# xiaojino/RUArt

Hardware: AMD Instinct MI355X
Metric: VQA samples/sec fwd+bwd (B=64, q=30, ocr=100) (higher is better)
Workload: dtype f16 MFMA + block-scaled fp8 (e4m3) MFMA correction, f32 accumulate / residual stream; 1 GPU; RUArt training step, synthetic ST-VQA-shaped batch: B=64/GPU, q=30 words, 100 OCR items, 36 objects, bert-base 12x768 frozen, SDNet trunk fwd+bwd, Adamax; global_batch=64, real_wordpieces_per_batch=42738, parallelism=dp1, mode=train

## Files before the change

### include/ruart_hip.h

```cpp
#ifndef RUART_HIP_H
#define RUART_HIP_H
#include <stddef.h>
#include <stdint.h>

#ifdef __cplusplus
extern "C" {
#endif

#define RUART_DT_F32 0
#define RUART_DT_BF16 1
#define RUART_DT_F16 2
#define RUART_ACT_NONE 0
#define RUART_ACT_GELU 1
#define RUART_ACT_RELU 2

const char* ruart_version(void);

int ruart_gemm_16_nt(const void* A, int lda, const void* W, int ldw, const float* bias, const void* residual, int ldr,
                     int residual_dtype, void* C, int ldc, int out_dtype, int M, int N, int K, int act, int in_dtype,
                     void* stream);
size_t ruart_gemm_16_tail_ws_bytes(int M, int N, int K, int cus);
int ruart_gemm_16_nt_ws(const void* A, int lda, const void* W, int ldw, const float* bias, const void* residual, int ldr, int residual_dtype,
                        void* C, int ldc, int out_dtype, int M, int N, int K, int act, int in_dtype, void* tail_ws, size_t tail_ws_bytes, int cus,
                        void* stream);
int ruart_gemm_16c_nt(const void* A16, const void* A8, int lda, const void* W16, const void* W8, int ldw, const float* bias,
                      const float* residual, int ldr, void* C, int ldc, void* C8, int M, int N, int K, int act, void* stream);
int ruart_f16c_shifts(int* out4);
int ruart_gemm_16c_set_dual(int on);
int ruart_gemm_16c_nt_sel(const void* A16, const void* A8, int lda, const void* W16, const void* W8, int ldw, const float* bias,
                          const float* residual, int ldr, void* C, int ldc, void* C8, int M, int N, int K, int act, int corr, void* stream);
size_t ruart_gemm_16c_tail_ws_bytes(int M, int N, int K, int cus);
int ruart_gemm_16c_nt_ws(const void* A16, const void* A8, int lda, const void* W16, const void* W8, int ldw, const float* bias,
                         const float* residual, int ldr, void* C, int ldc, void* C8, int M, int N, int K, int act, int corr, void* tail_ws,
                         size_t tail_ws_bytes, int cus, void* stream);
int ruart_gemm_16_nt_gelu2(const void* A, int lda, const void* W, int ldw, const float* bias, void* H16, void* G16, int ldc, int M, int N, int K,
                           int in_dtype, void* stream);
size_t ruart_gemm_16_nt_gelu_bwd_ws_floats(int M, int N);
int ruart_gemm_16_nt_gelu_bwd(const void* dY_bf16, int lda, const void* Wt_bf16, int ldw, const void* H16, int ldh, void* dH_bf16, void* G_bf16,
                              int ldc, float* colpart, int M, int N, int K, void* stream);
int ruart_gemm_16_nt_splitk(const void* A, int lda, const void* W, int ldw, float* part, int ldc, int M, int N, int K, int kchunk,
                            int in_dtype, void* stream);
int ruart_gemm_16_tn_splitk(const void* P, int ldp, const void* Q, int ldq, float* part, int ldc, int M, int N, int T, int tchunk,
                            int in_dtype, void* stream);
int ruart_gemm_set_tile_order(int group_m);
int ruart_gemm_set_variant(int v);
int ruart_gemm_f32_nt(const float* A, int lda, const float* W, int ldw, const float* bias, const float* residual, int ldr,
                      float* C, int ldc, int M, int N, int K, int act, void* stream);

int ruart_prof_enable(int on);
int ruart_prof_read(double* total_ms, long long* launches, double* flops);
int ruart_prof_mark(int tag, void* stream);
int ruart_prof_timeline(float* begin_ms, float* end_ms, double* flops, int max_records, int* n_records);

int ruart_bert_embed_ln(const int* ids, const int* pos_ids, const float* word_emb, const float* pos_emb, const float* type_emb,
                        const float* gamma, const float* beta, float eps, void* out, int ldo, int out_dtype, int rows, int H,
                        void* stream);
int ruart_rows_layernorm(const float* x, int ldx, const float* gamma, const float* beta, float eps, void* out, int ldo,
                         int out_dtype, int rows, int H, void* stream);
int ruart_rows_layernorm_split(const float* x, int ldx, const float* gamma, const float* beta, float eps, float* out32, void* out16,
                               void* out8, int ldo, int rows, int H, void* stream);
int ruart_bert_embed_ln_split(const int* ids, const int* pos_ids, const float* word_emb, const float* pos_emb, const float* type_emb,
                              const float* gamma, const float* beta, float eps, float* out32, void* out16, void* out8, int ldo, int rows,
                              int H, void* stream);
int ruart_bert_attention(const void* qkv, int ld, void* ctx, int ldc, int dtype, int H, int n_heads, int n_blocks,
                         const int* blk_q0, const int* blk_q1, const int* blk_k0, const int* blk_k1, const int* tok_lo,
                         const int* tok_hi, const float* key_bias, int n_long_blocks, const int* lblk_q0, const int* lblk_q1,
                         const int* lblk_k0, const int* lblk_k1, void* stream);
int ruart_bert_attention_split(const float* qkv, int ld, void* ctx16, void* ctx8, int ldc, int H, int n_heads, int n_blocks,
                               const int* blk_q0, const int* blk_q1, const int* blk_k0, const int* blk_k1, const int* tok_lo,
                               const int* tok_hi, const float* key_bias, void* stream);
int ruart_bert_attention_split_set_heads(int heads_per_workgroup);
int ruart_bert_pool_set_variant(int cols);
int ruart_bert_pool_mix(const void* layers, long long layer_stride, int ldl, int dtype, int n_layers, const int* span_start,
                        const int* span_start_last, const int* span_len, const int* dst_row, const float* layer_w, float* out, int ldo,
                        int n_words, int H, void* stream);
int ruart_bert_pool_mix_bwd(const void* layers, long long layer_stride, int ldl, int dtype, int n_layers, const int* span_start,
                            const int* span_start_last, const int* span_len, const int* dst_row, const float* grad_out, int ldg,
                            float* partial_ws, float* grad_layer_w, int n_words, int H, void* stream);
int ruart_rows_gather(const int* rows, int n, const void* src0, long long sp0, void* dst0, long long dp0, int bytes0, const void* src1,
                      long long sp1, void* dst1, long long dp1, int bytes1, const void* src2, long long sp2, void* dst2, long long dp2,
                      int bytes2, void* stream);
int ruart_cast_f32_to_16(const float* in, void* out, int out_dtype, long long n, float scale, void* stream);

int ruart_ln_train_fwd(const float* x, int ldx, const void* res16, int ldr, const float* gamma, const float* beta, float eps, float p,
                       unsigned seed, int post, void* y16, void* pre16, float* stats, int ld16, int rows, int H, void* stream);
size_t ruart_ln_train_bwd_ws_floats(int H);
int ruart_ln_train_bwd(const float* dy, int ldy, const float* add, const float* add_scale, const void* pre16, int ld16, const float* stats,
                       const float* gamma, float p, unsigned seed, int post, float* d_res, int ldd, void* d_gemm_bf16, int ldg,
                       float* d_gamma, float* d_beta, float* d_bias, int accumulate, float* ws, int rows, int H, void* stream);
typedef struct {
  const float* w;
  void* out16;
  void* outT_bf16;
  int ldw, ld16, ldT, rows, cols;
  float scale;
} ruart_wprep_item;
int ruart_weight_prep_batch(const ruart_wprep_item* items, int n, void* stream);
int ruart_weight_prep(const float* w, int ldw, float scale, void* out16, int ld16, void* outT_bf16, int ldT, int rows, int cols, void* stream);
size_t ruart_colsum_f32_ws_floats(int rows, int cols);
int ruart_colsum_f32(const float* x, int ld, int rows, int cols, float* out, int accumulate, float* ws, void* stream);
int ruart_colsum_f32_rows(const float* part, int rows, int ld, int cols, float* out, int accumulate, void* stream);
int ruart_gelu_bwd_rows(void* d_bf16, const void* h16, int ld, void* g_bf16, float* colpart, int M, int N, void* stream);
int ruart_f16_to_bf16(const void* in16, void* out_bf16, long long n, void* stream);
int ruart_colsum_bf16(const void* x_bf16, int ld, int rows, int cols, float* out, int accumulate, float* ws, void* stream);
int ruart_transpose16(const void* in, int ldi, void* out, int ldo, int rows, int cols, int f16_to_bf16, void* stream);
int ruart_splitk_reduce(const float* part, long long slab_floats, int nz, float* C, long long n, float scale, int accumulate, void* stream);
int ruart_mix_rows(const void* layers16, long long layer_stride, int ld, int n_layers, const float* w, float* out, int ldo, int rows, int H,
                   void* stream);
int ruart_mix_rows_bwd(const void* layers16, long long layer_stride, int ld, int n_layers, const float* g, int ldg, float* d_w, float* ws,
                       int rows, int H, void* stream);
int ruart_rows_ln_to_16(const float* y, long long layer_stride, int ldy, const float* ln_stats, long long stats_stride, const float* ln_gamma,
                        const float* ln_beta, void* out16, long long out_stride, int ldo, int n_layers, int n_tokens, int rows, int H,
                        void* stream);
int ruart_attn_train_fwd(const void* qkv16, int ld, void* ctx16, int ldc, int H, int n_heads, int n_blocks, const int* blk_q0,
                         const int* blk_q1, const int* tok_lo, float p_drop, unsigned seed, void* stream);
int ruart_attn_train_bwd(const void* qkv16, int ld, const void* dctx_bf16, int ldc, void* dqkv_bf16, int ldd, int H, int n_heads, int n_blocks,
                         const int* blk_q0, const int* blk_q1, const int* tok_lo, float p_drop, unsigned seed, float* bias_part, void* stream);
int ruart_attn_train_fwd_long(const void* qkv16, int ld, void* ctx16, int ldc, int H, int n_heads, int n_chunks, const int* chunk_q0,
                              const int* chunk_q1, const int* chunk_k0, const int* chunk_k1, float p_drop, unsigned seed, float* lse2,
                              void* stream);
int ruart_attn_train_bwd_long(const void* qkv16, int ld, const void* dctx_bf16, int ldc, void* dqkv_bf16, int ldd, int H, int n_heads,
                              int n_chunks, const int* chunk_q0, const int* chunk_q1, const int* chunk_k0, const int* chunk_k1, const int* chunk_first, float p_drop, unsigned seed, const float* lse2, float* delta_ws,
                              float* scale_ws, float* bias_part, void* stream);

typedef struct {
  int hidden, n_heads, n_layers, intermediate, dtype;
  float ln_eps;
  const float *word_emb, *pos_emb, *type_emb, *emb_ln_g, *emb_ln_b;
  const void* const* w_qkv;
  const float* const* b_qkv;
  const void* const* w_ao;    const float* const* b_ao;
  const float* const* ln1_g;  const float* const* ln1_b;
  const void* const* w_ff1;   const float* const* b_ff1;
  const void* const* w_ff2;   const float* const* b_ff2;
  const float* const* ln2_g;  const float* const* ln2_b;
  int f32_gemm;
  int corr8;
  const void* const* w8_qkv;
  const void* const* w8_ao;
  const void* const* w8_ff1;
  const void* const* w8_ff2;
  int tail_cus;
  int ln_fold;
  const float* const* fold_c_qkv;
  const float* const* fold_c_ff1;
  const float* fold_s_qkv;
  const float* fold_s_ff1;
} ruart_bert_model;

typedef struct {
  int n_tokens;
  int n_rows;
  const int* ids;
  const int* pos_ids;
  int n_blocks;
  const int *blk_q0, *blk_q1, *blk_k0, *blk_k1, *tok_lo, *tok_hi;
  const float* key_bias;
  int n_long_blocks;
  const int *lblk_q0, *lblk_q1, *lblk_k0, *lblk_k1;
  int n_last_rows;
  const int* last_rows;
} ruart_bert_batch;

size_t ruart_bert_workspace_bytes(const ruart_bert_model* m, int n_rows);
int ruart_bert_set_correction(int qkv, int ao, int ff1, int ff2, unsigned long long layer_mask);
int ruart_bert_forward(const ruart_bert_model* m, const ruart_bert_batch* b, void* layers_out, void* workspace,
                       size_t workspace_bytes, void* stream);

size_t ruart_bert_workspace_bytes_folded(const ruart_bert_model* m, int n_rows);
int ruart_bert_forward_folded(const ruart_bert_model* m, const ruart_bert_batch* b, void* layers_pre, float* ln_stats, void* workspace,
                              size_t workspace_bytes, void* stream);
int ruart_gemm_16c_nt_fold(const void* A16, const void* A8, int lda, const void* W16, const void* W8, int ldw, const float* bias, int kind,
                           const float* in_part, int in_np, const float* colc, float wscale, const float* residual, int ldr,
                           const float* res_part, int res_np, const float* res_gamma, const float* res_beta, void* C, int ldc, void* C16,
                           void* C8, float* out_part, int M, int N, int K, int stat_len, float eps, void* stream);
int ruart_gemm_16_nt_fold(const void* A, int lda, const void* W, int ldw, const float* bias, int kind, const float* in_part, int in_np,
                          const float* colc, float wscale, const void* residual, int ldr, const float* res_part, int res_np,
                          const float* res_gamma, const float* res_beta, void* C, int ldc, float* out_part, int M, int N, int K, int stat_len,
                          float eps, int dtype, void* stream);
int ruart_rows_stats_finish(const float* part, int np, int rows, float inv_h, float eps, float* stats, void* stream);
int ruart_bert_pool_mix_ln(const float* layers_pre, long long layer_stride, int ldl, int n_layers, const float* ln_stats,
                           long long stats_stride, const float* ln_gamma, const float* ln_beta, const int* span_start,
                           const int* span_start_last, const int* span_len, const int* dst_row, const float* layer_w, float* out, int ldo,
                           int n_words, int H, void* stream);
int ruart_bert_pool_ln_set_variant(int reg_tables);
int ruart_bert_pool_mix_ln_bwd(const float* layers_pre, long long layer_stride, int ldl, int n_layers, const float* ln_stats,
                               long long stats_stride, const float* ln_gamma, const float* ln_beta, const int* span_start,
                               const int* span_start_last, const int* span_len, const int* dst_row, const float* grad_out, int ldg,
                               float* partial_ws, float* grad_layer_w, int n_words, int H, void* stream);

int ruart_attn_fwd(const float* pa, const float* pk, const float* v, const unsigned char* mask, const float* diag, int diag_len,
                   int relu, float* out, float* probs, int B, int L1, int L2, int h, int D3, void* stream);
int ruart_attn_bwd(const float* pa, const float* pk, const float* v, const float* probs, const float* grad_out, const float* diag,
                   int diag_len, int relu, float* grad_pa, float* grad_pk, float* grad_v, float* grad_diag_partial,
                   float* ds_ws , int B, int L1, int L2, int h, int D3, void* stream);
int ruart_attn_set_prefetch(int on);
int ruart_attn_fwd_pscale(const float* pa, const float* pk, const float* v, const unsigned char* mask, const float* diag, int diag_len,
                          int relu, const float* prob_scale, float* out, float* probs, int B, int L1, int L2, int h, int D3,
                          void* stream);
int ruart_attn_bwd_pscale(const float* pa, const float* pk, const float* v, const float* probs, const float* grad_out, const float* diag,
                          int diag_len, int relu, const float* prob_scale, float* grad_pa, float* grad_pk, float* grad_v,
                          float* grad_diag_partial, float* ds_ws, int B, int L1, int L2, int h, int D3, void* stream);

int ruart_whole_ln_fwd(const float* x, float* y, float* stats, float* ws, long long n, float eps, void* stream);
int ruart_whole_ln_bwd(const float* y, const float* grad_y, const float* stats, float* grad_x, float* ws, long long n,
                       void* stream);

int ruart_whole_ln_blocks(void);
int ruart_whole_ln_partials(const float* x, const float* x2, float* part, long long n, void* stream);
int ruart_whole_ln_var_global(const float* x, long long n, const float* part_all, int world, long long n_total, float* part2,
                              void* stream);
int ruart_whole_ln_apply_global(const float* x, float* y, long long n, float eps, const float* part_all, const float* part2_all,
                                int world, long long n_total, float* stats, void* stream);
int ruart_whole_ln_bwd_global(const float* y, const float* grad_y, const float* stats, float* grad_x, long long n,
                              const float* part_all, int world, long long n_total, void* stream);

int ruart_scorer_fwd(const float* x, const float* u1, const float* u2, const float* uh, const float* w, const float* bna,
                     const unsigned char* mask, float* probs, float* a_out, int B, int L, int D, int ES, int mask_flag, void* stream);
int ruart_scorer_bwd(const float* x, const float* u1, const float* u2, const float* uh, const float* w, const float* probs,
                     const float* a_in, const float* gprobs, float* gx, float* gu1, float* gu2, float* guh, float* gw_part,
                     float* gb_part, int B, int L, int D, int ES, void* stream);

int ruart_scorer_heads_fwd(const float* x, const float* u1, const float* u2, const float* uh, const float* w, const float* bh,
                           const unsigned char* mask, float* probs, float* a_out, int B, int L, int D, int ES, int H, int n_front,
                           int mask_flag, void* stream);
int ruart_scorer_heads_bwd(const float* x, const float* u1, const float* u2, const float* uh, const float* w, const float* probs,
                           const float* a_in, const float* gprobs, float* gx, float* gu1, float* gu2, float* guh, float* gw_part,
                           float* gb_part, int B, int L, int D, int ES, int H, int n_front, void* stream);

int ruart_lstm_set_variant(int variant);
int ruart_lstm_ws_bytes(int h, int ndir, size_t* bytes);
int ruart_lstm_fwd(const float* xproj, const float* w_hh, float* y, float* gates, float* cells, float* hprev, int B, int T, int h,
                   int ndir, void* ws, size_t ws_bytes, void* stream);
int ruart_lstm_bwd(const float* grad_y, const float* w_hh, const float* gates, const float* cells, float* grad_xproj, int B,
                   int T, int h, int ndir, void* ws, size_t ws_bytes, void* stream);

int ruart_lstm_pack_params(const float* w_ih, const float* w_ih_r, const float* b_ih, const float* b_hh, const float* b_ih_r,
                           const float* b_hh_r, const float* w_hh, const float* w_hh_r, float* w, float* b, float* whh, int G, int K, int h,
                           void* stream);

int ruart_rows_scale(const float* x, int ldx, const float* mask, int ldm, const long long* row_of, float* out, int ldo, int rows, int D,
                     void* stream);
int ruart_lstm_cell_fwd(const float* pre, const float* h_prev, const float* c_prev, float* h_out, float* c_out, float* acts,
                        int n_active, int n_rows, int h, void* stream);
int ruart_lstm_cell_bwd(const float* grad_h, const float* grad_c, const float* acts, const float* c_prev, const float* c_out,
                        float* grad_pre, float* grad_h_prev, float* grad_c_prev, int n_active, int n_rows, int h, void* stream);

int ruart_embedding_bwd_sorted(const float* grad_out, const int* order, const int* seg_start, const int* seg_row, int n_seg, int D,
                               float* grad_weight, void* stream);
int ruart_embedding_bwd_split(const float* grad_out, const int* order, const int* sub_start, int n_sub, const int* row_first, const int* row_id,
                              int n_rows, int D, float* ws, float* grad_weight, void* stream);

int ruart_phoc_table(const unsigned char* chars, const int* offsets, int n_words, float* out, int ldo, int* status, void* stream);

#define RUART_EDIT_MAX_LEN 128
int ruart_edit_distance_pairs(const int32_t* chars, int n_chars, const int32_t* str_off, int n_str, const int32_t* pair_a,
                              const int32_t* pair_b, int n_pairs, int32_t* dist, int32_t* equal, void* stream);

int ruart_grad_norm_clip(const float* const* grads, const int* c_tensor, const int* c_start, const int* c_count, int n_chunks,
                         float max_norm, float* partial, float* norm_coef, const float* extra_sq, void* stream);
int ruart_adamax_step(float* const* params, const float* const* grads, float* const* exp_avg, float* const* exp_inf, const int* c_tensor,
                      const int* c_start, const int* c_count, int n_chunks, const float* norm_coef, const float* clr, float beta1,
                      float beta2, float eps, void* stream);
int ruart_adam_step(float* const* params, const float* const* grads, float* const* exp_avg, float* const* exp_avg_sq, const int* c_tensor,
                    const int* c_start, const int* c_count, int n_chunks, const float* norm_coef, const float* tab, float beta1,
                    float beta2, float eps, void* stream);

int ruart_set_nan_flag(int* flag);

int ruart_gemm_x3_plan(int M, int N, int K, int a_k_contiguous , int b_k_contiguous , int* splitk,
                       size_t* ws_bytes);
int ruart_gemm_x3(const float* A, long long sam, long long sak, const float* B, long long sbk, long long sbn, const float* bias,
                  const float* residual, int ldr, int act, float* C, int ldc, int M, int N, int K, float* ws, size_t ws_bytes,
                  const unsigned char* a_keep, const unsigned char* b_keep, float keep_scale, const float* c_scale, int rows_per_scale_row,
                  void* stream);
typedef struct {
  const float* A;
  const float* B;
  float* C;
  int lda, ldb, ldc, M, N, K, accumulate;
} ruart_x3_tn_problem;
size_t ruart_gemm_x3_tn_grouped_ws(const ruart_x3_tn_problem* probs, int n);
int ruart_gemm_x3_tn_grouped(const ruart_x3_tn_problem* probs, int n, float* ws, size_t ws_bytes, void* stream);
int ruart_gemm_x1(const float* A, long long sam, long long sak, const float* B, long long sbk, long long sbn, const float* bias,
                  const float* residual, int ldr, int act, float* C, int ldc, int M, int N, int K, float* ws, size_t ws_bytes,
                  const unsigned char* a_keep, const unsigned char* b_keep, float keep_scale, const float* c_scale, int rows_per_scale_row,
                  void* stream);

int ruart_gemm_bf16_tn(const float* A, long long sak_rows, const float* B, long long sbk_rows, float* C, int ldc, int M, int N, int K,
                       float* ws, size_t ws_bytes, void* stream);

int ruart_stream_create_cu_masked(int n_cus, void** stream_out);
int ruart_stream_create_priority(int priority, void** stream_out);
int ruart_stream_destroy(void* stream);

#ifdef __cplusplus
}
#endif
#endif
```

### ruart_amd/csrc/sdnet_attention.hip

```cpp
#include <cstdlib>
#include "common.h"
#include "ruart_hip.h"

#define CH 64
#define LDA_ 66
#define LDB_ 80
#define NTW 6
#define ATTN_MAX_L2 384

int* ruart_nan_flag_ptr = nullptr;

__device__ __forceinline__ f32x4_t mma16(const float* As, int lda, const float* Bs, int sbk, int sbj, int Kc, f32x4_t acc) {
  const int lane = threadIdx.x & 63, r = lane & 15, q = lane >> 4;
  for (int kk = 0; kk < Kc; kk += 4) acc = __builtin_amdgcn_mfma_f32_16x16x4f32(As[r * lda + kk + q], Bs[(kk + q) * sbk + r * sbj], acc, 0, 0, 0);
  return acc;
}

struct Act {
  int relu;
  const float* diag;
  int diag_len;
  __device__ __forceinline__ float operator()(float v, int col) const {
    if (relu) v = fmaxf(v, 0.f);
    if (diag_len == 1) v *= diag[0];
    else if (diag_len > 1) v *= diag[col];
    return v;
  }
};
__device__ __forceinline__ Act no_act() { return Act{0, nullptr, 0}; }

template <int U>
__device__ __forceinline__ void stage_u(float* dst, int ldd, int nr_pad, const float* src, int ld, int r0, int rows, int c0, int cols, Act act) {
  const int total = nr_pad * CH;
  for (int e0 = threadIdx.x; e0 < total; e0 += U * blockDim.x) {
    float v[U], dv[U];
    unsigned ok = 0;
#pragma unroll
    for (int u = 0; u < U; ++u) {
      const int e = e0 + u * blockDim.x;
      const int r = e / CH, c = e % CH;
      const int gr = r0 + r, gc = c0 + c;
      if (e < total && gr < rows && gc < cols) ok |= 1u << u;
      v[u] = src[(size_t)min(gr, rows - 1) * ld + min(gc, cols - 1)];
    }
    if (act.diag_len > 1) {
#pragma unroll
      for (int u = 0; u < U; ++u) dv[u] = act.diag[min(c0 + (e0 + u * (int)blockDim.x) % CH, cols - 1)];
    } else {
      const float d1 = act.diag_len == 1 ? act.diag[0] : 1.f;
#pragma unroll
      for (int u = 0; u < U; ++u) dv[u] = d1;
    }
#pragma unroll
    for (int u = 0; u < U; ++u) {
      const int e = e0 + u * blockDim.x;
      float x = v[u];
      if (act.relu) x = fmaxf(x, 0.f);
      x *= dv[u];
      if (e < total) dst[(e / CH) * ldd + (e % CH)] = ((ok >> u) & 1u) ? x : 0.f;
    }
  }
}
__device__ __forceinline__ void stage(float* dst, int ldd, int nr_pad, const float* src, int ld, int r0, int rows, int c0, int cols,
                                      Act act = Act{0, nullptr, 0}) {
  if (nr_pad <= 16) stage_u<4>(dst, ldd, nr_pad, src, ld, r0, rows, c0, cols, act);
  else if (nr_pad <= 32) stage_u<8>(dst, ldd, nr_pad, src, ld, r0, rows, c0, cols, act);
  else stage_u<16>(dst, ldd, nr_pad, src, ld, r0, rows, c0, cols, act);
}
__device__ __forceinline__ void stage_t16(float* dst, int ldd, const float* src, int ld, int r0, int rows, int c0, int cols,
                                          const float* mul = nullptr) {
  float v[4], m[4];
  unsigned ok = 0;
#pragma unroll
  for (int u = 0; u < 4; ++u) {
    const int e = threadIdx.x + u * 256;
    const int c = e & 15, r = e >> 4;
    const int gr = r0 + r, gc = c0 + c;
    if (gr < rows && gc < cols) ok |= 1u << u;
    const size_t at = (size_t)min(gr, rows - 1) * ld + min(gc, cols - 1);
    v[u] = src[at];
    m[u] = mul ? mul[at] : 1.f;
  }
#pragma unroll
  for (int u = 0; u < 4; ++u) {
    const int e = threadIdx.x + u * 256;
    dst[(e & 15) * ldd + (e >> 4)] = ((ok >> u) & 1u) ? v[u] * m[u] : 0.f;
  }
}

__device__ __forceinline__ int lds_probs_stride(int L2p) { return ((L2p + 31) / 32) * 32 + 2; }

extern __shared__ __attribute__((aligned(16))) float dsm[];

__global__ __launch_bounds__(256) void attn_fwd_kernel(const float* __restrict__ a, const float* __restrict__ k,
                                                       const float* __restrict__ v, const unsigned char* __restrict__ mask,
                                                       float* __restrict__ out, float* __restrict__ probs, int L1, int L2, int h,
                                                       int D3, int* __restrict__ nan_flag, int relu, const float* __restrict__ diag,
                                                       int diag_len, const float* __restrict__ pscale) {
  const int b = blockIdx.y, i0 = blockIdx.x * 16;
  const int lane = threadIdx.x & 63, wave = threadIdx.x >> 6;
  const int L2p = (L2 + 15) & ~15, ldS = lds_probs_stride(L2p);
  float* a_s = dsm;
  float* S_s = a_s + 16 * LDA_;
  float* kv_s = S_s + 16 * ldS;
  const float* ab = a + (size_t)b * L1 * h;
  const float* kb = k + (size_t)b * L2 * h;
  const float* vb = v + (size_t)b * L2 * D3;
  const int ntile = L2p / 16;

  f32x4_t acc[NTW];
#pragma unroll
  for (int t = 0; t < NTW; ++t) acc[t] = (f32x4_t){0.f, 0.f, 0.f, 0.f};
  for (int c0 = 0; c0 < h; c0 += CH) {
    __syncthreads();
    stage(a_s, LDA_, 16, ab, h, i0, L1, c0, h, Act{relu, diag, diag_len});
    stage(kv_s, LDA_, L2p, kb, h, 0, L2, c0, h, Act{relu, nullptr, 0});
    __syncthreads();
    const int kc = min(CH, (h - c0 + 3) & ~3);
#pragma unroll
    for (int t = 0; t < NTW; ++t) {
      const int jt = wave + 4 * t;
      if (jt < ntile) acc[t] = mma16(a_s, LDA_, kv_s + jt * 16 * LDA_, 1, LDA_, kc, acc[t]);
    }
  }
#pragma unroll
  for (int t = 0; t < NTW; ++t) {
    const int jt = wave + 4 * t;
    if (jt < ntile) {
#pragma unroll
      for (int r = 0; r < 4; ++r) S_s[((lane >> 4) * 4 + r) * ldS + jt * 16 + (lane & 15)] = acc[t][r];
    }
  }
  __syncthreads();
  {
    const int row = threadIdx.x >> 4, c = threadIdx.x & 15;
    const unsigned char* mb = mask + (size_t)b * L2;
    float* Sr = S_s + row * ldS;
    float mx = -INFINITY;
    for (int j = c; j < L2; j += 16) {
      const float s = mb[j] ? Sr[j] : -INFINITY;
      Sr[j] = s;
      mx = fmaxf(mx, s);
    }
#pragma unroll
    for (int o = 8; o > 0; o >>= 1) mx = fmaxf(mx, __shfl_xor(mx, o, 64));
    float sum = 0.f;
    for (int j = c; j < L2; j += 16) {
      const float e = expf(Sr[j] - mx);
      Sr[j] = e;
      sum += e;
    }
#pragma unroll
    for (int o = 8; o > 0; o >>= 1) sum += __shfl_xor(sum, o, 64);
    const float inv = 1.0f / sum;
    const bool live = (i0 + row) < L1;
    bool bad = false;
    for (int j = c; j < L2p; j += 16) {
      const float p = (j < L2) ? Sr[j] * inv : 0.f;
      const float ps = (pscale && live && j < L2) ? pscale[((size_t)b * L1 + i0 + row) * L2 + j] : 1.f;
      Sr[j] = live ? p * ps : 0.f;
      bad |= live && !(p == p);
      if (probs && live && j < L2) probs[((size_t)b * L1 + i0 + row) * L2 + j] = p;
    }
    if (bad && nan_flag) atomicOr(nan_flag, 1);
  }
  for (int d0 = 0; d0 < D3; d0 += CH) {
    __syncthreads();
    stage(kv_s, LDB_, L2p, vb, D3, 0, L2, d0, D3);
    __syncthreads();
    f32x4_t o = {0.f, 0.f, 0.f, 0.f};
    o = mma16(S_s, ldS, kv_s + wave * 16, LDB_, 1, L2p, o);
    const int d = d0 + wave * 16 + (lane & 15);
#pragma unroll
    for (int r = 0; r < 4; ++r) {
      const int i = i0 + (lane >> 4) * 4 + r;
      if (i < L1 && d < D3) out[((size_t)b * L1 + i) * D3 + d] = o[r];
    }
  }
}

__global__ __launch_bounds__(256) void attn_bwd_q_kernel(const float* __restrict__ k, const float* __restrict__ v,
                                                         const float* __restrict__ probs, const float* __restrict__ gout,
                                                         float* __restrict__ grad_a, float* __restrict__ dS, int L1, int L2, int h,
                                                         int D3, const float* __restrict__ pa, int relu,
                                                         const float* __restrict__ diag, int diag_len,
                                                         float* __restrict__ grad_diag, const float* __restrict__ pscale) {
  const int b = blockIdx.y, i0 = blockIdx.x * 16;
  const int lane = threadIdx.x & 63, wave = threadIdx.x >> 6;
  const int L2p = (L2 + 15) & ~15, ldS = lds_probs_stride(L2p);
  float* g_s = dsm;
  float* S_s = g_s + 16 * LDA_;
  float* kv_s = S_s + 16 * ldS;
  const float* kb = k + (size_t)b * L2 * h;
  const float* vb = v + (size_t)b * L2 * D3;
  const float* gb = gout + (size_t)b * L1 * D3;
  const int ntile = L2p / 16;

  f32x4_t acc[NTW];
#pragma unroll
  for (int t = 0; t < NTW; ++t) acc[t] = (f32x4_t){0.f, 0.f, 0.f, 0.f};
  for (int c0 = 0; c0 < D3; c0 += CH) {
    __syncthreads();
    stage(g_s, LDA_, 16, gb, D3, i0, L1, c0, D3);
    stage(kv_s, LDA_, L2p, vb, D3, 0, L2, c0, D3);
    __syncthreads();
    const int kc = min(CH, (D3 - c0 + 3) & ~3);
#pragma unroll
    for (int t = 0; t < NTW; ++t) {
      const int jt = wave + 4 * t;
      if (jt < ntile) acc[t] = mma16(g_s, LDA_, kv_s + jt * 16 * LDA_, 1, LDA_, kc, acc[t]);
    }
  }
#pragma unroll
  for (int t = 0; t < NTW; ++t) {
    const int jt = wave + 4 * t;
    if (jt < ntile) {
#pragma unroll
      for (int r = 0; r < 4; ++r) S_s[((lane >> 4) * 4 + r) * ldS + jt * 16 + (lane & 15)] = acc[t][r];
    }
  }
  __syncthreads();
  {
    const int row = threadIdx.x >> 4, c = threadIdx.x & 15;
    const bool live = (i0 + row) < L1;
    const float* Pr = probs + ((size_t)b * L1 + (live ? i0 + row : 0)) * L2;
    float* Sr = S_s + row * ldS;
    float dot = 0.f;
    if (pscale && live) {
      const float* Mr = pscale + ((size_t)b * L1 + i0 + row) * L2;
      for (int j = c; j < L2; j += 16) Sr[j] *= Mr[j];
    }
    for (int j = c; j < L2; j += 16) dot += Sr[j] * Pr[j];
#pragma unroll
    for (int o = 8; o > 0; o >>= 1) dot += __shfl_xor(dot, o, 64);
    for (int j = c; j < L2p; j += 16) {
      float d = 0.f;
      if (live && j < L2) {
        const float p = Pr[j];
        d = p * (Sr[j] - dot);
        dS[((size_t)b * L1 + i0 + row) * L2 + j] = d;
      }
      Sr[j] = d;
    }
  }
  for (int d0 = 0; d0 < h; d0 += CH) {
    __syncthreads();
    stage(kv_s, LDB_, L2p, kb, h, 0, L2, d0, h, Act{relu, nullptr, 0});
    __syncthreads();
    f32x4_t o = {0.f, 0.f, 0.f, 0.f};
    o = mma16(S_s, ldS, kv_s + wave * 16, LDB_, 1, L2p, o);
    const int d = d0 + wave * 16 + (lane & 15);
    float gd = 0.f;
    const float dsc = (d < h) ? (diag_len == 1 ? diag[0] : (diag_len > 1 ? diag[d] : 1.f)) : 0.f;
#pragma unroll
    for (int r = 0; r < 4; ++r) {
      const int i = i0 + (lane >> 4) * 4 + r;
      if (i < L1 && d < h) {
        const size_t at = ((size_t)b * L1 + i) * h + d;
        float g = o[r];
        if (pa) {
          const float pv = pa[at];
          gd += g * (relu ? fmaxf(pv, 0.f) : pv);
          g = (relu && pv <= 0.f) ? 0.f : g * dsc;
        }
        grad_a[at] = g;
      }
    }
    if (grad_diag) {
      gd += __shfl_xor(gd, 16, 64);
      gd += __shfl_xor(gd, 32, 64);
      if ((lane >> 4) == 0 && d < h) grad_diag[((size_t)b * gridDim.x + blockIdx.x) * h + d] = gd;
    }
  }
}

__device__ __forceinline__ void tn_product(const float* X, int L1, int L2, int j0, const float* Y, int N, float* C, float* xt_s,
                                           float* y_s, Act yact, const float* out_gate, const float* xmul = nullptr) {
  const int lane = threadIdx.x & 63, wave = threadIdx.x >> 6;
  for (int n0 = 0; n0 < N; n0 += CH) {
    f32x4_t o = {0.f, 0.f, 0.f, 0.f};
    for (int r0 = 0; r0 < L1; r0 += CH) {
      __syncthreads();
      stage_t16(xt_s, LDA_, X, L2, r0, L1, j0, L2, xmul);
      stage(y_s, LDB_, CH, Y, N, r0, L1, n0, N, yact);
      __syncthreads();
      const int kc = min(CH, (L1 - r0 + 3) & ~3);
      o = mma16(xt_s, LDA_, y_s + wave * 16, LDB_, 1, kc, o);
    }
    const int n = n0 + wave * 16 + (lane & 15);
#pragma unroll
    for (int r = 0; r < 4; ++r) {
      const int j = j0 + (lane >> 4) * 4 + r;
      if (j < L2 && n < N) {
        const size_t at = (size_t)j * N + n;
        C[at] = (out_gate && out_gate[at] <= 0.f) ? 0.f : o[r];
      }
    }
  }
}

__global__ __launch_bounds__(256) void attn_bwd_kv_kernel(const float* __restrict__ a, const float* __restrict__ probs,
                                                          const float* __restrict__ dS, const float* __restrict__ gout,
                                                          float* __restrict__ grad_k, float* __restrict__ grad_v, int L1, int L2, int h,
                                                          int D3, const float* __restrict__ pk, int relu,
                                                          const float* __restrict__ diag, int diag_len,
                                                          const float* __restrict__ pscale) {
  const int b = blockIdx.y, j0 = blockIdx.x * 16;
  float* xt_s = dsm;
  float* y_s = xt_s + 16 * LDA_;
  const size_t pb = (size_t)b * L1 * L2;
  tn_product(dS + pb, L1, L2, j0, a + (size_t)b * L1 * h, h, grad_k + (size_t)b * L2 * h, xt_s, y_s, Act{relu, diag, diag_len},
             (relu && pk) ? pk + (size_t)b * L2 * h : nullptr);
  tn_product(probs + pb, L1, L2, j0, gout + (size_t)b * L1 * D3, D3, grad_v + (size_t)b * L2 * D3, xt_s, y_s, no_act(), nullptr,
             pscale ? pscale + pb : nullptr);
}

template <int U, bool DIAG = false>
struct Panel {
  float v[U];
  float dv[DIAG ? U : 1];
  unsigned ok;
  __device__ __forceinline__ void load(const float* __restrict__ src, int ld, int nr_pad, int r0, int rows, int c0, int cols,
                                       const float* __restrict__ diag = nullptr, int diag_len = 0) {
    ok = 0;
    const int total = nr_pad * CH;
#pragma unroll
    for (int u = 0; u < U; ++u) {
      const int e = (int)threadIdx.x + u * 256;
      const int r = e / CH, c = e % CH;
      const int gr = r0 + r, gc = c0 + c;
      if (e < total && gr < rows && gc < cols) ok |= 1u << u;
      v[u] = src[(size_t)min(gr, rows - 1) * ld + min(gc, cols - 1)];
      if (DIAG) dv[u] = diag_len > 1 ? diag[min(gc, cols - 1)] : (diag_len == 1 ? diag[0] : 1.f);
    }
  }
  __device__ __forceinline__ void store(float* dst, int ldd, int nr_pad, int relu) const {
    const int total = nr_pad * CH;
#pragma unroll
    for (int u = 0; u < U; ++u) {
      const int e = (int)threadIdx.x + u * 256;
      float x = v[u];
      if (relu) x = fmaxf(x, 0.f);
      x *= DIAG ? dv[u] : 1.f;
      if (e < total) dst[(e / CH) * ldd + (e % CH)] = ((ok >> u) & 1u) ? x : 0.f;
    }
  }
};

template <int UK>
__global__ __launch_bounds__(256) void attn_fwd_pf_kernel(const float* __restrict__ a, const float* __restrict__ k,
                                                          const float* __restrict__ v, const unsigned char* __restrict__ mask,
                                                          float* __restrict__ out, float* __restrict__ probs, int L1, int L2, int h,
                                                          int D3, int* __restrict__ nan_flag, int relu, const float* __restrict__ diag,
                                                          int diag_len, const float* __restrict__ pscale) {
  const int b = blockIdx.y, i0 = blockIdx.x * 16;
  const int lane = threadIdx.x & 63, wave = threadIdx.x >> 6;
  const int L2p = (L2 + 15) & ~15, ldS = lds_probs_stride(L2p);
  float* a_s = dsm;
  float* S_s = a_s + 16 * LDA_;
  float* kv_s = S_s + 16 * ldS;
  const float* ab = a + (size_t)b * L1 * h;
  const float* kb = k + (size_t)b * L2 * h;
  const float* vb = v + (size_t)b * L2 * D3;
  const int ntile = L2p / 16;

  Panel<4, true> pa;
  Panel<UK> pk;
  pa.load(ab, h, 16, i0, L1, 0, h, diag, diag_len);
  pk.load(kb, h, L2p, 0, L2, 0, h);
  f32x4_t acc[NTW];
#pragma unroll
  for (int t = 0; t < NTW; ++t) acc[t] = (f32x4_t){0.f, 0.f, 0.f, 0.f};
  for (int c0 = 0; c0 < h; c0 += CH) {
    __syncthreads();
    pa.store(a_s, LDA_, 16, relu);
    pk.store(kv_s, LDA_, L2p, relu);
    {
      const bool more = c0 + CH < h;
      pa.load(ab, h, 16, i0, L1, more ? c0 + CH : 0, h, diag, diag_len);
      pk.load(more ? kb : vb, more ? h : D3, L2p, 0, L2, more ? c0 + CH : 0, more ? h : D3);
    }
    __syncthreads();
    const int kc = min(CH, (h - c0 + 3) & ~3);
#pragma unroll
    for (int t = 0; t < NTW; ++t) {
      const int jt = wave + 4 * t;
      if (jt < ntile) acc[t] = mma16(a_s, LDA_, kv_s + jt * 16 * LDA_, 1, LDA_, kc, acc[t]);
    }
  }
#pragma unroll
  for (int t = 0; t < NTW; ++t) {
    const int jt = wave + 4 * t;
    if (jt < ntile) {
#pragma unroll
      for (int r = 0; r < 4; ++r) S_s[((lane >> 4) * 4 + r) * ldS + jt * 16 + (lane & 15)] = acc[t][r];
    }
  }
  __syncthreads();
  {
    const int row = threadIdx.x >> 4, c = threadIdx.x & 15;
    const unsigned char* mb = mask + (size_t)b * L2;
    float* Sr = S_s + row * ldS;
    float mx = -INFINITY;
    for (int j = c; j < L2; j += 16) {
      const float s = mb[j] ? Sr[j] : -INFINITY;
      Sr[j] = s;
      mx = fmaxf(mx, s);
    }
#pragma unroll
    for (int o = 8; o > 0; o >>= 1) mx = fmaxf(mx, __shfl_xor(mx, o, 64));
    float sum = 0.f;
    for (int j = c; j < L2; j += 16) {
      const float e = expf(Sr[j] - mx);
      Sr[j] = e;
      sum += e;
    }
#pragma unroll
    for (int o = 8; o > 0; o >>= 1) sum += __shfl_xor(sum, o, 64);
    const float inv = 1.0f / sum;
    const bool live = (i0 + row) < L1;
    bool bad = false;
    for (int j = c; j < L2p; j += 16) {
      const float p = (j < L2) ? Sr[j] * inv : 0.f;
      const float ps = (pscale && live && j < L2) ? pscale[((size_t)b * L1 + i0 + row) * L2 + j] : 1.f;
      Sr[j] = live ? p * ps : 0.f;
      bad |= live && !(p == p);
      if (probs && live && j < L2) probs[((size_t)b * L1 + i0 + row) * L2 + j] = p;
    }
    if (bad && nan_flag) atomicOr(nan_flag, 1);
  }
  for (int d0 = 0; d0 < D3; d0 += CH) {
    __syncthreads();
    pk.store(kv_s, LDB_, L2p, 0);
    pk.load(vb, D3, L2p, 0, L2, d0 + CH < D3 ? d0 + CH : 0, D3);
    __syncthreads();
    f32x4_t o = {0.f, 0.f, 0.f, 0.f};
    o = mma16(S_s, ldS, kv_s + wave * 16, LDB_, 1, L2p, o);
    const int d = d0 + wave * 16 + (lane & 15);
#pragma unroll
    for (int r = 0; r < 4; ++r) {
      const int i = i0 + (lane >> 4) * 4 + r;
      if (i < L1 && d < D3) out[((size_t)b * L1 + i) * D3 + d] = o[r];
    }
  }
}

template <int UK>
__global__ __launch_bounds__(256) void attn_bwd_q_pf_kernel(const float* __restrict__ k, const float* __restrict__ v,
                                                            const float* __restrict__ probs, const float* __restrict__ gout,
                                                            float* __restrict__ grad_a, float* __restrict__ dS, int L1, int L2, int h,
                                                            int D3, const float* __restrict__ pa_, int relu,
                                                            const float* __restrict__ diag, int diag_len,
                                                            float* __restrict__ grad_diag, const float* __restrict__ pscale) {
  const int b = blockIdx.y, i0 = blockIdx.x * 16;
  const int lane = threadIdx.x & 63, wave = threadIdx.x >> 6;
  const int L2p = (L2 + 15) & ~15, ldS = lds_probs_stride(L2p);
  float* g_s = dsm;
  float* S_s = g_s + 16 * LDA_;
  float* kv_s = S_s + 16 * ldS;
  const float* kb = k + (size_t)b * L2 * h;
  const float* vb = v + (size_t)b * L2 * D3;
  const float* gb = gout + (size_t)b * L1 * D3;
  const int ntile = L2p / 16;

  Panel<4> pg;
  Panel<UK> pk;
  pg.load(gb, D3, 16, i0, L1, 0, D3);
  pk.load(vb, D3, L2p, 0, L2, 0, D3);
  f32x4_t acc[NTW];
#pragma unroll
  for (int t = 0; t < NTW; ++t) acc[t] = (f32x4_t){0.f, 0.f, 0.f, 0.f};
  for (int c0 = 0; c0 < D3; c0 += CH) {
    __syncthreads();
    pg.store(g_s, LDA_, 16, 0);
    pk.store(kv_s, LDA_, L2p, 0);
    {
      const bool more = c0 + CH < D3;
      pg.load(gb, D3, 16, i0, L1, more ? c0 + CH : 0, D3);
      pk.load(more ? vb : kb, more ? D3 : h, L2p, 0, L2, more ? c0 + CH : 0, more ? D3 : h);
    }
    __syncthreads();
    const int kc = min(CH, (D3 - c0 + 3) & ~3);
#pragma unroll
    for (int t = 0; t < NTW; ++t) {
      const int jt = wave + 4 * t;
      if (jt < ntile) acc[t] = mma16(g_s, LDA_, kv_s + jt * 16 * LDA_, 1, LDA_, kc, acc[t]);
    }
  }
#pragma unroll
  for (int t = 0; t < NTW; ++t) {
    const int jt = wave + 4 * t;
    if (jt < ntile) {
#pragma unroll
      for (int r = 0; r < 4; ++r) S_s[((lane >> 4) * 4 + r) * ldS + jt * 16 + (lane & 15)] = acc[t][r];
    }
  }
  __syncthreads();
  {
    const int row = threadIdx.x >> 4, c = threadIdx.x & 15;
    const bool live = (i0 + row) < L1;
    const float* Pr = probs + ((size_t)b * L1 + (live ? i0 + row : 0)) * L2;
    float* Sr = S_s + row * ldS;
    float dot = 0.f;
    if (pscale && live) {
      const float* Mr = pscale + ((size_t)b * L1 + i0 + row) * L2;
      for (int j = c; j < L2; j += 16) Sr[j] *= Mr[j];
    }
    for (int j = c; j < L2; j += 16) dot += Sr[j] * Pr[j];
#pragma unroll
    for (int o = 8; o > 0; o >>= 1) dot += __shfl_xor(dot, o, 64);
    for (int j = c; j < L2p; j += 16) {
      float d = 0.f;
      if (live && j < L2) {
        const float p = Pr[j];
        d = p * (Sr[j] - dot);
        dS[((size_t)b * L1 + i0 + row) * L2 + j] = d;
      }
      Sr[j] = d;
    }
  }
  for (int d0 = 0; d0 < h; d0 += CH) {
    __syncthreads();
    pk.store(kv_s, LDB_, L2p, relu);
    pk.load(kb, h, L2p, 0, L2, d0 + CH < h ? d0 + CH : 0, h);
    __syncthreads();
    f32x4_t o = {0.f, 0.f, 0.f, 0.f};
    o = mma16(S_s, ldS, kv_s + wave * 16, LDB_, 1, L2p, o);
    const int d = d0 + wave * 16 + (lane & 15);
    float gd = 0.f;
    const float dsc = (d < h) ? (diag_len == 1 ? diag[0] : (diag_len > 1 ? diag[d] : 1.f)) : 0.f;
#pragma unroll
    for (int r = 0; r < 4; ++r) {
      const int i = i0 + (lane >> 4) * 4 + r;
      if (i < L1 && d < h) {
        const size_t at = ((size_t)b * L1 + i) * h + d;
        float g = o[r];
        if (pa_) {
          const float pv = pa_[at];
          gd += g * (relu ? fmaxf(pv, 0.f) : pv);
          g = (relu && pv <= 0.f) ? 0.f : g * dsc;
        }
        grad_a[at] = g;
      }
    }
    if (grad_diag) {
      gd += __shfl_xor(gd, 16, 64);
      gd += __shfl_xor(gd, 32, 64);
      if ((lane >> 4) == 0 && d < h) grad_diag[((size_t)b * gridDim.x + blockIdx.x) * h + d] = gd;
    }
  }
}

struct PanelT16 {
  float v[4], m[4];
  unsigned ok;
  __device__ __forceinline__ void load(const float* __restrict__ src, int ld, int r0, int rows, int c0, int cols, const float* __restrict__ mul) {
    ok = 0;
#pragma unroll
    for (int u = 0; u < 4; ++u) {
      const int e = (int)threadIdx.x + u * 256;
      const int c = e & 15, r = e >> 4;
      const int gr = r0 + r, gc = c0 + c;
      if (gr < rows && gc < cols) ok |= 1u << u;
      const size_t at = (size_t)min(gr, rows - 1) * ld + min(gc, cols - 1);
      v[u] = src[at];
      m[u] = mul ? mul[at] : 1.f;
    }
  }
  __device__ __forceinline__ void store(float* dst, int ldd) const {
#pragma unroll
    for (int u = 0; u < 4; ++u) {
      const int e = (int)threadIdx.x + u * 256;
      dst[(e & 15) * ldd + (e >> 4)] = ((ok >> u) & 1u) ? v[u] * m[u] : 0.f;
    }
  }
};

__device__ __forceinline__ void tn_product_pf(const float* X, int L1, int L2, int j0, const float* Y, int N, float* C, float* xt_s,
                                              float* y_s, Act yact, const float* out_gate, const float* xmul) {
  const int lane = threadIdx.x & 63, wave = threadIdx.x >> 6;
  const int nr = (L1 + CH - 1) / CH, nn = (N + CH - 1) / CH, steps = nr * nn;
  PanelT16 px;
  Panel<16, true> py;
  px.load(X, L2, 0, L1, j0, L2, xmul);
  py.load(Y, N, CH, 0, L1, 0, N, yact.diag, yact.diag_len);
  f32x4_t o = {0.f, 0.f, 0.f, 0.f};
  int ri = 0, ni = 0;
  for (int s = 0; s < steps; ++s) {
    const int r0 = ri * CH, n0 = ni * CH;
    __syncthreads();
    px.store(xt_s, LDA_);
    py.store(y_s, LDB_, CH, yact.relu);
    int rn = ri + 1, nx = ni;
    if (rn == nr) { rn = 0; nx = ni + 1; }
    if (nx == nn) { rn = 0; nx = 0; }
    px.load(X, L2, rn * CH, L1, j0, L2, xmul);
    py.load(Y, N, CH, rn * CH, L1, nx * CH, N, yact.diag, yact.diag_len);
    __syncthreads();
    const int kc = min(CH, (L1 - r0 + 3) & ~3);
    o = mma16(xt_s, LDA_, y_s + wave * 16, LDB_, 1, kc, o);
    if (ri == nr - 1) {
      const int n = n0 + wave * 16 + (lane & 15);
#pragma unroll
      for (int r = 0; r < 4; ++r) {
        const int j = j0 + (lane >> 4) * 4 + r;
        if (j < L2 && n < N) {
          const size_t at = (size_t)j * N + n;
          C[at] = (out_gate && out_gate[at] <= 0.f) ? 0.f : o[r];
        }
      }
      o = (f32x4_t){0.f, 0.f, 0.f, 0.f};
    }
    ri = rn;
    ni = nx;
  }
}

__global__ __launch_bounds__(256) void attn_bwd_kv_pf_kernel(const float* __restrict__ a, const float* __restrict__ probs,
                                                             const float* __restrict__ dS, const float* __restrict__ gout,
                                                             float* __restrict__ grad_k, float* __restrict__ grad_v, int L1, int L2, int h,
                                                             int D3, const float* __restrict__ pk, int relu,
                                                             const float* __restrict__ diag, int diag_len,
                                                             const float* __restrict__ pscale) {
  const int b = blockIdx.y, j0 = blockIdx.x * 16;
  float* xt_s = dsm;
  float* y_s = xt_s + 16 * LDA_;
  const size_t pb = (size_t)b * L1 * L2;
  tn_product_pf(dS + pb, L1, L2, j0, a + (size_t)b * L1 * h, h, grad_k + (size_t)b * L2 * h, xt_s, y_s, Act{relu, diag, diag_len},
                (relu && pk) ? pk + (size_t)b * L2 * h : nullptr, nullptr);
  tn_product_pf(probs + pb, L1, L2, j0, gout + (size_t)b * L1 * D3, D3, grad_v + (size_t)b * L2 * D3, xt_s, y_s, no_act(), nullptr,
                pscale ? pscale + pb : nullptr);
}

#define WLN_BLOCKS 256
__device__ __forceinline__ float grid_partial_total(const float* part, float* red) {
  float s = (threadIdx.x < WLN_BLOCKS) ? part[threadIdx.x] : 0.f;
  return block_sum<4>(s, red);
}

#define WLN_FOR4(n4, ...)                                                                          \
  for (long long i_ = blockIdx.x * 256LL + threadIdx.x; i_ < (n4); i_ += 4LL * 256 * WLN_BLOCKS) { \
    long long ix_[4];                                                                              \
    bool ok_[4];                                                                                   \
    _Pragma("unroll") for (int u_ = 0; u_ < 4; ++u_) {                                             \
      const long long j_ = i_ + (long long)u_ * 256 * WLN_BLOCKS;                                  \
      ok_[u_] = j_ < (n4);                                                                         \
      ix_[u_] = ok_[u_] ? j_ : (n4) - 1;                                                           \
    }                                                                                              \
    __VA_ARGS__                                                                                    \
  }
__device__ __forceinline__ bool wln_vec_ok(const void* a, const void* b, const void* c, long long n) {
  return ((n & 3) == 0) && (((reinterpret_cast<uintptr_t>(a) | reinterpret_cast<uintptr_t>(b) | reinterpret_cast<uintptr_t>(c)) & 15) == 0) && n >= 4;
}

__global__ __launch_bounds__(256) void wln_sum_kernel(const float* __restrict__ x, const float* __restrict__ x2, long long n,
                                                      float* __restrict__ part) {
  __shared__ float red[4];
  float s = 0.f, t = 0.f;
  if (wln_vec_ok(x, x2, nullptr, n)) {
    const f32x4_t* x4 = reinterpret_cast<const f32x4_t*>(x);
    const f32x4_t* y4 = reinterpret_cast<const f32x4_t*>(x2);
    const long long n4 = n >> 2;
    if (x2) {
      WLN_FOR4(n4, f32x4_t a[4], b[4];
               _Pragma("unroll") for (int u = 0; u < 4; ++u) { a[u] = x4[ix_[u]]; b[u] = y4[ix_[u]]; }
               _Pragma("unroll") for (int u = 0; u < 4; ++u) if (ok_[u]) {
                 s += (a[u][0] + a[u][1]) + (a[u][2] + a[u][3]);
                 t += (a[u][0] * b[u][0] + a[u][1] * b[u][1]) + (a[u][2] * b[u][2] + a[u][3] * b[u][3]);
               })
    } else {
      WLN_FOR4(n4, f32x4_t a[4];
               _Pragma("unroll") for (int u = 0; u < 4; ++u) a[u] = x4[ix_[u]];
               _Pragma("unroll") for (int u = 0; u < 4; ++u) if (ok_[u]) s += (a[u][0] + a[u][1]) + (a[u][2] + a[u][3]);)
    }
  } else {
    for (long long i = blockIdx.x * 256LL + threadIdx.x; i < n; i += 256LL * WLN_BLOCKS) {
      const float a = x[i];
      s += a;
      if (x2) t += a * x2[i];
    }
  }
  s = block_sum<4>(s, red);
  if (x2) t = block_sum<4>(t, red);
  if (threadIdx.x == 0) {
    part[blockIdx.x] = s;
    if (x2) part[WLN_BLOCKS + blockIdx.x] = t;
  }
}
__global__ __launch_bounds__(256) void wln_var_kernel(const float* __restrict__ x, long long n, const float* __restrict__ part,
                                                      float* __restrict__ part2) {
  __shared__ float red[4];
  const float mean = grid_partial_total(part, red) / (float)n;
  float q = 0.f;
  if (wln_vec_ok(x, nullptr, nullptr, n)) {
    const f32x4_t* x4 = reinterpret_cast<const f32x4_t*>(x);
    const long long n4 = n >> 2;
    WLN_FOR4(n4, f32x4_t a[4];
             _Pragma("unroll") for (int u = 0; u < 4; ++u) a[u] = x4[ix_[u]];
             _Pragma("unroll") for (int u = 0; u < 4; ++u) if (ok_[u]) {
               const f32x4_t d = a[u] - mean;
               q += (d[0] * d[0] + d[1] * d[1]) + (d[2] * d[2] + d[3] * d[3]);
             })
  } else {
    for (long long i = blockIdx.x * 256LL + threadIdx.x; i < n; i += 256LL * WLN_BLOCKS) {
      const float d = x[i] - mean;
      q += d * d;
    }
  }
  q = block_sum<4>(q, red);
  if (threadIdx.x == 0) part2[blockIdx.x] = q;
}
__global__ __launch_bounds__(256) void wln_apply_kernel(const float* __restrict__ x, float* __restrict__ y, long long n, float eps,
                                                        const float* __restrict__ part, const float* __restrict__ part2,
                                                        float* __restrict__ stats, int* __restrict__ nan_flag) {
  __shared__ float red[4];
  const float mean = grid_partial_total(part, red) / (float)n;
  const float var = grid_partial_total(part2, red) / (float)n;
  const float rstd = 1.0f / sqrtf(var + eps);
  if (blockIdx.x == 0 && threadIdx.x == 0) {
    stats[0] = mean;
    stats[1] = rstd;
  }
  bool bad = false;
  if (wln_vec_ok(x, y, nullptr, n)) {
    const f32x4_t* x4 = reinterpret_cast<const f32x4_t*>(x);
    f32x4_t* y4 = reinterpret_cast<f32x4_t*>(y);
    const long long n4 = n >> 2;
    WLN_FOR4(n4, f32x4_t a[4];
             _Pragma("unroll") for (int u = 0; u < 4; ++u) a[u] = x4[ix_[u]];
             _Pragma("unroll") for (int u = 0; u < 4; ++u) if (ok_[u]) {
               const f32x4_t o = (a[u] - mean) * rstd;
               y4[ix_[u]] = o;
               bad |= !(o[0] == o[0]) || !(o[1] == o[1]) || !(o[2] == o[2]) || !(o[3] == o[3]);
             })
  } else {
    for (long long i = blockIdx.x * 256LL + threadIdx.x; i < n; i += 256LL * WLN_BLOCKS) {
      const float o = (x[i] - mean) * rstd;
      y[i] = o;
      bad |= !(o == o);
    }
  }
  if (bad && nan_flag) atomicOr(nan_flag, 1);
}
__global__ __launch_bounds__(256) void wln_bwd_kernel(const float* __restrict__ y, const float* __restrict__ gy,
                                                      const float* __restrict__ stats, float* __restrict__ gx, long long n,
                                                      const float* __restrict__ part) {
  __shared__ float red[4];
  const float mg = grid_partial_total(part, red) / (float)n;
  const float mgy = grid_partial_total(part + WLN_BLOCKS, red) / (float)n;
  const float rstd = stats[1];
  if (wln_vec_ok(y, gy, gx, n)) {
    const f32x4_t* y4 = reinterpret_cast<const f32x4_t*>(y);
    const f32x4_t* g4 = reinterpret_cast<const f32x4_t*>(gy);
    f32x4_t* o4 = reinterpret_cast<f32x4_t*>(gx);
    const long long n4 = n >> 2;
    WLN_FOR4(n4, f32x4_t a[4], b[4];
             _Pragma("unroll") for (int u = 0; u < 4; ++u) { a[u] = y4[ix_[u]]; b[u] = g4[ix_[u]]; }
             _Pragma("unroll") for (int u = 0; u < 4; ++u) if (ok_[u]) o4[ix_[u]] = rstd * (b[u] - mg - a[u] * mgy);)
  } else {
    for (long long i = blockIdx.x * 256LL + threadIdx.x; i < n; i += 256LL * WLN_BLOCKS) gx[i] = rstd * (gy[i] - mg - y[i] * mgy);
  }
}

__device__ __forceinline__ float wln_ranks_total(const float* part, int stride, int world, float* red) {
  float t = grid_partial_total(part, red);
  for (int r = 1; r < world; ++r) t += grid_partial_total(part + (long long)r * stride, red);
  return t;
}
__global__ __launch_bounds__(256) void wln_var_global_kernel(const float* __restrict__ x, long long n, const float* __restrict__ part_all,
                                                             int world, long long n_total, float* __restrict__ part2) {
  __shared__ float red[4];
  const float mean = wln_ranks_total(part_all, WLN_BLOCKS, world, red) / (float)n_total;
  float q = 0.f;
  if (wln_vec_ok(x, nullptr, nullptr, n)) {
    const f32x4_t* x4 = reinterpret_cast<const f32x4_t*>(x);
    const long long n4 = n >> 2;
    WLN_FOR4(n4, f32x4_t a[4];
             _Pragma("unroll") for (int u = 0; u < 4; ++u) a[u] = x4[ix_[u]];
             _Pragma("unroll") for (int u = 0; u < 4; ++u) if (ok_[u]) {
               const f32x4_t d = a[u] - mean;
               q += (d[0] * d[0] + d[1] * d[1]) + (d[2] * d[2] + d[3] * d[3]);
             })
  } else {
    for (long long i = blockIdx.x * 256LL + threadIdx.x; i < n; i += 256LL * WLN_BLOCKS) {
      const float d = x[i] - mean;
      q += d * d;
    }
  }
  q = block_sum<4>(q, red);
  if (threadIdx.x == 0) part2[blockIdx.x] = q;
}
__global__ __launch_bounds__(256) void wln_apply_global_kernel(const float* __restrict__ x, float* __restrict__ y, long long n, float eps,
                                                               const float* __restrict__ part_all, const float* __restrict__ part2_all,
                                                               int world, long long n_total, float* __restrict__ stats,
                                                               int* __restrict__ nan_flag) {
  __shared__ float red[4];
  const float mean = wln_ranks_total(part_all, WLN_BLOCKS, world, red) / (float)n_total;
  const float var = wln_ranks_total(part2_all, WLN_BLOCKS, world, red) / (float)n_total;
  const float rstd = 1.0f / sqrtf(var + eps);
  if (blockIdx.x == 0 && threadIdx.x == 0) {
    stats[0] = mean;
    stats[1] = rstd;
  }
  bool bad = false;
  if (wln_vec_ok(x, y, nullptr, n)) {
    const f32x4_t* x4 = reinterpret_cast<const f32x4_t*>(x);
    f32x4_t* y4 = reinterpret_cast<f32x4_t*>(y);
    const long long n4 = n >> 2;
    WLN_FOR4(n4, f32x4_t a[4];
             _Pragma("unroll") for (int u = 0; u < 4; ++u) a[u] = x4[ix_[u]];
             _Pragma("unroll") for (int u = 0; u < 4; ++u) if (ok_[u]) {
               const f32x4_t o = (a[u] - mean) * rstd;
               y4[ix_[u]] = o;
               bad |= !(o[0] == o[0]) || !(o[1] == o[1]) || !(o[2] == o[2]) || !(o[3] == o[3]);
             })
  } else {
    for (long long i = blockIdx.x * 256LL + threadIdx.x; i < n; i += 256LL * WLN_BLOCKS) {
      const float o = (x[i] - mean) * rstd;
      y[i] = o;
      bad |= !(o == o);
    }
  }
  if (bad && nan_flag) atomicOr(nan_flag, 1);
}
__global__ __launch_bounds__(256) void wln_bwd_global_kernel(const float* __restrict__ y, const float* __restrict__ gy,
                                                             const float* __restrict__ stats, float* __restrict__ gx, long long n,
                                                             const float* __restrict__ part_all, int world, long long n_total) {
  __shared__ float red[4];
  const float mg = wln_ranks_total(part_all, 2 * WLN_BLOCKS, world, red) / (float)n_total;
  const float mgy = wln_ranks_total(part_all + WLN_BLOCKS, 2 * WLN_BLOCKS, world, red) / (float)n_total;
  const float rstd = stats[1];
  if (wln_vec_ok(y, gy, gx, n)) {
    const f32x4_t* y4 = reinterpret_cast<const f32x4_t*>(y);
    const f32x4_t* g4 = reinterpret_cast<const f32x4_t*>(gy);
    f32x4_t* o4 = reinterpret_cast<f32x4_t*>(gx);
    const long long n4 = n >> 2;
    WLN_FOR4(n4, f32x4_t a[4], b[4];
             _Pragma("unroll") for (int u = 0; u < 4; ++u) { a[u] = y4[ix_[u]]; b[u] = g4[ix_[u]]; }
             _Pragma("unroll") for (int u = 0; u < 4; ++u) if (ok_[u]) o4[ix_[u]] = rstd * (b[u] - mg - a[u] * mgy);)
  } else {
    for (long long i = blockIdx.x * 256LL + threadIdx.x; i < n; i += 256LL * WLN_BLOCKS) gx[i] = rstd * (gy[i] - mg - y[i] * mgy);
  }
}

static bool g_attn_prefetch = !(getenv("RUART_ATTN_PREFETCH") && atoi(getenv("RUART_ATTN_PREFETCH")) == 0);
template <typename K> static void attn_big_lds(K kern) { hipFuncSetAttribute((const void*)kern, hipFuncAttributeMaxDynamicSharedMemorySize, 160 * 1024); }
static void attn_allow_big_lds() {
  static bool done = (attn_big_lds(attn_fwd_kernel), attn_big_lds(attn_bwd_q_kernel), attn_big_lds(attn_fwd_pf_kernel<12>),
                      attn_big_lds(attn_fwd_pf_kernel<16>), attn_big_lds(attn_fwd_pf_kernel<28>), attn_big_lds(attn_fwd_pf_kernel<32>),
                      attn_big_lds(attn_bwd_q_pf_kernel<12>), attn_big_lds(attn_bwd_q_pf_kernel<16>), attn_big_lds(attn_bwd_q_pf_kernel<28>),
                      attn_big_lds(attn_bwd_q_pf_kernel<32>), true);
  (void)done;
}

static size_t attn_lds_bytes(int L2) {
  const int L2p = (L2 + 15) & ~15;
  const int ldS = ((L2p + 31) / 32) * 32 + 2;
  return sizeof(float) * (size_t)(16 * LDA_ + 16 * ldS + L2p * LDB_);
}

__global__ __launch_bounds__(256) void attn1_fwd_kernel(const float* __restrict__ a, const float* __restrict__ k,
                                                        const float* __restrict__ v, const unsigned char* __restrict__ mask,
                                                        float* __restrict__ out, float* __restrict__ probs, int L2, int h, int D3,
                                                        int* __restrict__ nan_flag) {
  __shared__ float p_s[ATTN_MAX_L2];
  __shared__ float red[4];
  const int b = blockIdx.x, tid = threadIdx.x, lane = tid & 63, wave = tid >> 6;
  const float* ab = a + (size_t)b * h;
  const float* kb = k + (size_t)b * L2 * h;
  const float* vb = v + (size_t)b * L2 * D3;
  for (int j0 = wave * 4; j0 < L2; j0 += 16) {
    float s[4] = {0.f, 0.f, 0.f, 0.f};
    for (int d = lane; d < h; d += 64) {
      const float av = ab[d];
#pragma unroll
      for (int u = 0; u < 4; ++u)
        if (j0 + u < L2) s[u] = fmaf(av, kb[(size_t)(j0 + u) * h + d], s[u]);
    }
#pragma unroll
    for (int u = 0; u < 4; ++u) {
      const float t = wave_sum(s[u]);
      if (lane == 0 && j0 + u < L2) p_s[j0 + u] = mask[(size_t)b * L2 + j0 + u] ? t : -INFINITY;
    }
  }
  __syncthreads();
  float mx = -INFINITY;
  for (int j = tid; j < L2; j += 256) mx = fmaxf(mx, p_s[j]);
  mx = block_max<4>(mx, red);
  float sum = 0.f;
  for (int j = tid; j < L2; j += 256) {
    const float e = expf(p_s[j] - mx);
    p_s[j] = e;
    sum += e;
  }
  sum = block_sum<4>(sum, red);
  __syncthreads();
  const float inv = 1.0f / sum;
  bool bad = false;
  for (int j = tid; j < L2; j += 256) {
    const float p = p_s[j] * inv;
    p_s[j] = p;
    bad |= !(p == p);
    if (probs) probs[(size_t)b * L2 + j] = p;
  }
  if (bad && nan_flag) atomicOr(nan_flag, 1);
  __syncthreads();
  for (int d = tid; d < D3; d += 256) {
    float o = 0.f;
    int j = 0;
    for (; j + 8 <= L2; j += 8) {
      float t[8];
#pragma unroll
      for (int u = 0; u < 8; ++u) t[u] = vb[(size_t)(j + u) * D3 + d];
#pragma unroll
      for (int u = 0; u < 8; ++u) o = fmaf(p_s[j + u], t[u], o);
    }
    for (; j < L2; ++j) o = fmaf(p_s[j], vb[(size_t)j * D3 + d], o);
    out[(size_t)b * D3 + d] = o;
  }
}

__global__ __launch_bounds__(256) void attn1_bwd_kernel(const float* __restrict__ a, const float* __restrict__ k,
                                                        const float* __restrict__ v, const float* __restrict__ probs,
                                                        const float* __restrict__ gout, float* __restrict__ grad_a,
                                                        float* __restrict__ grad_k, float* __restrict__ grad_v, int L2, int h, int D3) {
  __shared__ float ds_s[ATTN_MAX_L2];
  __shared__ float red[4];
  const int b = blockIdx.x, tid = threadIdx.x, lane = tid & 63, wave = tid >> 6;
  const float* ab = a + (size_t)b * h;
  const float* kb = k + (size_t)b * L2 * h;
  const float* vb = v + (size_t)b * L2 * D3;
  const float* gb = gout + (size_t)b * D3;
  const float* pb = probs + (size_t)b * L2;
  for (int j0 = wave * 4; j0 < L2; j0 += 16) {
    float s[4] = {0.f, 0.f, 0.f, 0.f};
    for (int d = lane; d < D3; d += 64) {
      const float gv = gb[d];
#pragma unroll
      for (int u = 0; u < 4; ++u)
        if (j0 + u < L2) s[u] = fmaf(gv, vb[(size_t)(j0 + u) * D3 + d], s[u]);
    }
#pragma unroll
    for (int u = 0; u < 4; ++u) {
      const float t = wave_sum(s[u]);
      if (lane == 0 && j0 + u < L2) ds_s[j0 + u] = t;
    }
  }
  __syncthreads();
  float dot = 0.f;
  for (int j = tid; j < L2; j += 256) dot += ds_s[j] * pb[j];
  dot = block_sum<4>(dot, red);
  __syncthreads();
  for (int j = tid; j < L2; j += 256) ds_s[j] = pb[j] * (ds_s[j] - dot);
  __syncthreads();
  for (int d = tid; d < h; d += 256) {
    float g = 0.f;
    int j = 0;
    for (; j + 8 <= L2; j += 8) {
      float t[8];
#pragma unroll
      for (int u = 0; u < 8; ++u) t[u] = kb[(size_t)(j + u) * h + d];
#pragma unroll
      for (int u = 0; u < 8; ++u) g = fmaf(ds_s[j + u], t[u], g);
    }
    for (; j < L2; ++j) g = fmaf(ds_s[j], kb[(size_t)j * h + d], g);
    grad_a[(size_t)b * h + d] = g;
  }
  for (int e = tid; e < L2 * h; e += 256) grad_k[(size_t)b * L2 * h + e] = ds_s[e / h] * ab[e % h];
  for (int e = tid; e < L2 * D3; e += 256) grad_v[(size_t)b * L2 * D3 + e] = pb[e / D3] * gb[e % D3];
}

extern "C" int ruart_attn_fwd(const float* a, const float* k, const float* v, const unsigned char* mask, const float* diag,
                              int diag_len, int relu, float* out, float* probs, int B, int L1, int L2, int h, int D3, void* stream) {
  RUART_ENTRY();
  return ruart_attn_fwd_pscale(a, k, v, mask, diag, diag_len, relu, nullptr, out, probs, B, L1, L2, h, D3, stream);
}

extern "C" int ruart_attn_fwd_pscale(const float* a, const float* k, const float* v, const unsigned char* mask, const float* diag,
                                     int diag_len, int relu, const float* prob_scale, float* out, float* probs, int B, int L1, int L2,
                                     int h, int D3, void* stream) {
  RUART_ENTRY();
  if (B <= 0 || L1 <= 0 || L2 <= 0 || L2 > ATTN_MAX_L2 || h <= 0 || D3 <= 0) return (int)hipErrorInvalidValue;
  if (diag_len != 0 && diag_len != 1 && diag_len != h) return (int)hipErrorInvalidValue;
  if (L1 == 1 && !relu && diag_len == 0 && !prob_scale) {
    hipLaunchKernelGGL(attn1_fwd_kernel, dim3(B), dim3(256), 0, (hipStream_t)stream, a, k, v, mask, out, probs, L2, h, D3,
                       ruart_nan_flag_ptr);
    RUART_CHECK_LAUNCH();
    return 0;
  }
  const dim3 grid(ceil_div(L1, 16), B), block(256);
  attn_allow_big_lds();
  const int L2p = (L2 + 15) & ~15;
#define RUART_AF(U) hipLaunchKernelGGL(attn_fwd_pf_kernel<U>, grid, block, attn_lds_bytes(L2), (hipStream_t)stream, a, k, v, mask, out, probs, \
                                       L1, L2, h, D3, ruart_nan_flag_ptr, relu, diag_len ? diag : nullptr, diag_len, prob_scale)
  if (!g_attn_prefetch || L2p > 128)
    hipLaunchKernelGGL(attn_fwd_kernel, grid, block, attn_lds_bytes(L2), (hipStream_t)stream, a, k, v, mask, out, probs, L1, L2, h, D3,
                       ruart_nan_flag_ptr, relu, diag_len ? diag : nullptr, diag_len, prob_scale);
  else if (L2p <= 48) RUART_AF(12);
  else if (L2p <= 64) RUART_AF(16);
  else if (L2p <= 112) RUART_AF(28);
  else RUART_AF(32);
#undef RUART_AF
  RUART_CHECK_LAUNCH();
  return 0;
}

extern "C" int ruart_attn_set_prefetch(int on) {
  RUART_ENTRY();
  g_attn_prefetch = on != 0;
  return 0;
}

extern "C" int ruart_attn_bwd(const float* a, const float* k, const float* v, const float* probs, const float* grad_out,
                              const float* diag, int diag_len, int relu, float* grad_a, float* grad_k, float* grad_v,
                              float* grad_diag, float* ds_ws, int B, int L1, int L2, int h, int D3, void* stream) {
  RUART_ENTRY();
  return ruart_attn_bwd_pscale(a, k, v, probs, grad_out, diag, diag_len, relu, nullptr, grad_a, grad_k, grad_v, grad_diag, ds_ws, B, L1,
                               L2, h, D3, stream);
}

extern "C" int ruart_attn_bwd_pscale(const float* a, const float* k, const float* v, const float* probs, const float* grad_out,
                                     const float* diag, int diag_len, int relu, const float* prob_scale, float* grad_a, float* grad_k,
                                     float* grad_v, float* grad_diag, float* ds_ws, int B, int L1, int L2, int h, int D3,
                                     void* stream) {
  RUART_ENTRY();
  if (B <= 0 || L1 <= 0 || L2 <= 0 || L2 > ATTN_MAX_L2 || h <= 0 || D3 <= 0) return (int)hipErrorInvalidValue;
  if (diag_len != 0 && diag_len != 1 && diag_len != h) return (int)hipErrorInvalidValue;
  if (L1 == 1 && !relu && diag_len == 0 && !prob_scale) {
    hipLaunchKernelGGL(attn1_bwd_kernel, dim3(B), dim3(256), 0, (hipStream_t)stream, a, k, v, probs, grad_out, grad_a, grad_k, grad_v,
                       L2, h, D3);
    RUART_CHECK_LAUNCH();
    return 0;
  }
  const bool act = relu || diag_len;
  const float* dg = diag_len ? diag : nullptr;
  attn_allow_big_lds();
  const int L2p = (L2 + 15) & ~15;
#define RUART_AQ(U) hipLaunchKernelGGL(attn_bwd_q_pf_kernel<U>, dim3(ceil_div(L1, 16), B), dim3(256), attn_lds_bytes(L2), (hipStream_t)stream, \
                                       k, v, probs, grad_out, grad_a, ds_ws, L1, L2, h, D3, act ? a : nullptr, relu, dg, diag_len,           \
                                       (diag_len > 1) ? grad_diag : nullptr, prob_scale)
  if (!g_attn_prefetch || L2p > 128)
    hipLaunchKernelGGL(attn_bwd_q_kernel, dim3(ceil_div(L1, 16), B), dim3(256), attn_lds_bytes(L2), (hipStream_t)stream, k, v, probs,
                       grad_out, grad_a, ds_ws, L1, L2, h, D3, act ? a : nullptr, relu, dg, diag_len,
                       (diag_len > 1) ? grad_diag : nullptr, prob_scale);
  else if (L2p <= 48) RUART_AQ(12);
  else if (L2p <= 64) RUART_AQ(16);
  else if (L2p <= 112) RUART_AQ(28);
  else RUART_AQ(32);
#undef RUART_AQ
  RUART_CHECK_LAUNCH();
  const size_t lds = sizeof(float) * (16 * LDA_ + CH * LDB_);
  if (g_attn_prefetch)
    hipLaunchKernelGGL(attn_bwd_kv_pf_kernel, dim3(ceil_div(L2, 16), B), dim3(256), lds, (hipStream_t)stream, a, probs, ds_ws, grad_out,
                       grad_k, grad_v, L1, L2, h, D3, k, relu, dg, diag_len, prob_scale);
  else
    hipLaunchKernelGGL(attn_bwd_kv_kernel, dim3(ceil_div(L2, 16), B), dim3(256), lds, (hipStream_t)stream, a, probs, ds_ws, grad_out,
                       grad_k, grad_v, L1, L2, h, D3, k, relu, dg, diag_len, prob_scale);
  RUART_CHECK_LAUNCH();
  return 0;
}

extern "C" int ruart_whole_ln_fwd(const float* x, float* y, float* stats, float* ws, long long n, float eps, void* stream) {
  RUART_ENTRY();
  if (n <= 0) return (int)hipErrorInvalidValue;
  hipStream_t s = (hipStream_t)stream;
  hipLaunchKernelGGL(wln_sum_kernel, dim3(WLN_BLOCKS), dim3(256), 0, s, x, (const float*)nullptr, n, ws);
  hipLaunchKernelGGL(wln_var_kernel, dim3(WLN_BLOCKS), dim3(256), 0, s, x, n, ws, ws + 2 * WLN_BLOCKS);
  hipLaunchKernelGGL(wln_apply_kernel, dim3(WLN_BLOCKS), dim3(256), 0, s, x, y, n, eps, ws, ws + 2 * WLN_BLOCKS, stats, ruart_nan_flag_ptr);
  RUART_CHECK_LAUNCH();
  return 0;
}

extern "C" int ruart_whole_ln_bwd(const float* y, const float* grad_y, const float* stats, float* grad_x, float* ws, long long n,
                                  void* stream) {
  RUART_ENTRY();
  if (n <= 0) return (int)hipErrorInvalidValue;
  hipStream_t s = (hipStream_t)stream;
  hipLaunchKernelGGL(wln_sum_kernel, dim3(WLN_BLOCKS), dim3(256), 0, s, grad_y, y, n, ws);
  hipLaunchKernelGGL(wln_bwd_kernel, dim3(WLN_BLOCKS), dim3(256), 0, s, y, grad_y, stats, grad_x, n, ws);
  RUART_CHECK_LAUNCH();
  return 0;
}

extern "C" int ruart_whole_ln_blocks(void) { return WLN_BLOCKS; }

extern "C" int ruart_whole_ln_partials(const float* x, const float* x2, float* part, long long n, void* stream) {
  RUART_ENTRY();
  if (n <= 0 || !x || !part) return (int)hipErrorInvalidValue;
  hipLaunchKernelGGL(wln_sum_kernel, dim3(WLN_BLOCKS), dim3(256), 0, (hipStream_t)stream, x, x2, n, part);
  RUART_CHECK_LAUNCH();
  return 0;
}

extern "C" int ruart_whole_ln_var_global(const float* x, long long n, const float* part_all, int world, long long n_total, float* part2,
                                         void* stream) {
  RUART_ENTRY();
  if (n <= 0 || world < 1 || n_total < n) return (int)hipErrorInvalidValue;
  hipLaunchKernelGGL(wln_var_global_kernel, dim3(WLN_BLOCKS), dim3(256), 0, (hipStream_t)stream, x, n, part_all, world, n_total, part2);
  RUART_CHECK_LAUNCH();
  return 0;
}

extern "C" int ruart_whole_ln_apply_global(const float* x, float* y, long long n, float eps, const float* part_all, const float* part2_all,
                                           int world, long long n_total, float* stats, void* stream) {
  RUART_ENTRY();
  if (n <= 0 || world < 1 || n_total < n) return (int)hipErrorInvalidValue;
  hipLaunchKernelGGL(wln_apply_global_kernel, dim3(WLN_BLOCKS), dim3(256), 0, (hipStream_t)stream, x, y, n, eps, part_all, part2_all, world,
                     n_total, stats, ruart_nan_flag_ptr);
  RUART_CHECK_LAUNCH();
  return 0;
}

extern "C" int ruart_whole_ln_bwd_global(const float* y, const float* grad_y, const float* stats, float* grad_x, long long n,
                                         const float* part_all, int world, long long n_total, void* stream) {
  RUART_ENTRY();
  if (n <= 0 || world < 1 || n_total < n) return (int)hipErrorInvalidValue;
  hipLaunchKernelGGL(wln_bwd_global_kernel, dim3(WLN_BLOCKS), dim3(256), 0, (hipStream_t)stream, y, grad_y, stats, grad_x, n, part_all,
                     world, n_total);
  RUART_CHECK_LAUNCH();
  return 0;
}

extern "C" int ruart_stream_create_cu_masked(int n_cus, void** stream_out) {
  RUART_ENTRY();
  if (!stream_out) return -1;
  int dev = 0, total = 0;
  if (hipGetDevice(&dev) != hipSuccess) return -2;
  if (hipDeviceGetAttribute(&total, hipDeviceAttributeMultiprocessorCount, dev) != hipSuccess) return -2;
  hipStream_t s = nullptr;
  hipError_t e;
  if (n_cus < 0 && -n_cus < total) {
    uint32_t mask[16] = {0};
    for (int i = total + n_cus; i < total && i < 512; ++i) mask[i >> 5] |= 1u << (i & 31);
    e = hipExtStreamCreateWithCUMask(&s, (uint32_t)((total + 31) / 32), mask);
  } else if (n_cus <= 0 || n_cus >= total) {
    e = hipStreamCreateWithFlags(&s, hipStreamNonBlocking);
  } else {
    uint32_t mask[16] = {0};
    for (int i = 0; i < n_cus && i < 512; ++i) mask[i >> 5] |= 1u << (i & 31);
    e = hipExtStreamCreateWithCUMask(&s, (uint32_t)((total + 31) / 32), mask);
  }
  if (e != hipSuccess) return -3;
  *stream_out = (void*)s;
  return 0;
}

extern "C" int ruart_stream_create_priority(int priority, void** stream_out) {
  RUART_ENTRY();
  if (!stream_out) return -1;
  int least = 0, greatest = 0;
  if (hipDeviceGetStreamPriorityRange(&least, &greatest) != hipSuccess) return -2;
  if (priority > least) priority = least;
  if (priority < greatest) priority = greatest;
  hipStream_t s = nullptr;
  if (hipStreamCreateWithPriority(&s, hipStreamNonBlocking, priority) != hipSuccess) return -3;
  *stream_out = (void*)s;
  return priority - greatest;
}

extern "C" int ruart_stream_destroy(void* stream) {
  RUART_ENTRY();
  return hipStreamDestroy((hipStream_t)stream) == hipSuccess ? 0 : -1;
}

extern "C" int ruart_set_nan_flag(int* flag) {
  RUART_ENTRY();
  ruart_nan_flag_ptr = flag;
  return 0;
}
```

### ruart_amd/hip.py

```python
import ctypes
import os
from ctypes import POINTER, Structure, c_char_p, c_double, c_float, c_int, c_longlong, c_size_t, c_uint, c_ulonglong, c_void_p

import torch

_HERE = os.path.dirname(os.path.abspath(__file__))
LIB_PATH = os.path.join(_HERE, "libruart_hip.so")

DT_F32, DT_BF16, DT_F16 = 0, 1, 2
ACT_NONE, ACT_GELU, ACT_RELU = 0, 1, 2
TORCH_DTYPE = {DT_F32: torch.float32, DT_BF16: torch.bfloat16, DT_F16: torch.float16}
PRECISION = {"fp32": DT_F32, "bf16": DT_BF16, "fp16": DT_F16, "x3": DT_F32, "fp16c": DT_F32}


class BertModelC(Structure):
    _fields_ = [("hidden", c_int), ("n_heads", c_int), ("n_layers", c_int), ("intermediate", c_int), ("dtype", c_int),
                ("ln_eps", c_float),
                ("word_emb", c_void_p), ("pos_emb", c_void_p), ("type_emb", c_void_p), ("emb_ln_g", c_void_p), ("emb_ln_b", c_void_p),
                ("w_qkv", POINTER(c_void_p)), ("b_qkv", POINTER(c_void_p)),
                ("w_ao", POINTER(c_void_p)), ("b_ao", POINTER(c_void_p)),
                ("ln1_g", POINTER(c_void_p)), ("ln1_b", POINTER(c_void_p)),
                ("w_ff1", POINTER(c_void_p)), ("b_ff1", POINTER(c_void_p)),
                ("w_ff2", POINTER(c_void_p)), ("b_ff2", POINTER(c_void_p)),
                ("ln2_g", POINTER(c_void_p)), ("ln2_b", POINTER(c_void_p)), ("f32_gemm", c_int), ("corr8", c_int),
                ("w8_qkv", POINTER(c_void_p)), ("w8_ao", POINTER(c_void_p)), ("w8_ff1", POINTER(c_void_p)), ("w8_ff2", POINTER(c_void_p)),
                ("tail_cus", c_int), ("ln_fold", c_int), ("fold_c_qkv", POINTER(c_void_p)), ("fold_c_ff1", POINTER(c_void_p)),
                ("fold_s_qkv", POINTER(c_float)), ("fold_s_ff1", POINTER(c_float))]


class X3TnProblemC(Structure):
    _fields_ = [("A", c_void_p), ("B", c_void_p), ("C", c_void_p), ("lda", c_int), ("ldb", c_int), ("ldc", c_int), ("M", c_int), ("N", c_int),
                ("K", c_int), ("accumulate", c_int)]


class WPrepItemC(Structure):
    _fields_ = [("w", c_void_p), ("out16", c_void_p), ("outT_bf16", c_void_p), ("ldw", c_int), ("ld16", c_int), ("ldT", c_int), ("rows", c_int),
                ("cols", c_int), ("scale", c_float)]


class BertBatchC(Structure):
    _fields_ = [("n_tokens", c_int), ("n_rows", c_int), ("ids", c_void_p), ("pos_ids", c_void_p), ("n_blocks", c_int),
                ("blk_q0", c_void_p), ("blk_q1", c_void_p), ("blk_k0", c_void_p), ("blk_k1", c_void_p),
                ("tok_lo", c_void_p), ("tok_hi", c_void_p), ("key_bias", c_void_p),
                ("n_long_blocks", c_int), ("lblk_q0", c_void_p), ("lblk_q1", c_void_p), ("lblk_k0", c_void_p), ("lblk_k1", c_void_p),
                ("n_last_rows", c_int), ("last_rows", c_void_p)]


class TensorPtr(c_void_p):

    @classmethod
    def from_param(cls, v):
        if isinstance(v, torch.Tensor):
            return c_void_p(v.data_ptr())
        if v is None:
            return c_void_p()
        if isinstance(v, c_void_p):
            return v
        if isinstance(v, int):
            return c_void_p(v)
        return super().from_param(v)


_P, _I, _F, _LL, _SZ, _U = TensorPtr, c_int, c_float, c_longlong, c_size_t, c_uint
_SIGNATURES = {
    "ruart_version": (c_char_p, []),
    "ruart_gemm_16_nt": (_I, [_P, _I, _P, _I, _P, _P, _I, _I, _P, _I, _I, _I, _I, _I, _I, _I, _P]),
    "ruart_gemm_16_tail_ws_bytes": (_SZ, [_I, _I, _I, _I]),
    "ruart_gemm_16_nt_ws": (_I, [_P, _I, _P, _I, _P, _P, _I, _I, _P, _I, _I, _I, _I, _I, _I, _I, _P, _SZ, _I, _P]),
    "ruart_gemm_16c_nt": (_I, [_P, _P, _I, _P, _P, _I, _P, _P, _I, _P, _I, _P, _I, _I, _I, _I, _P]),
    "ruart_gemm_16c_nt_sel": (_I, [_P, _P, _I, _P, _P, _I, _P, _P, _I, _P, _I, _P, _I, _I, _I, _I, _I, _P]),
    "ruart_gemm_16c_tail_ws_bytes": (_SZ, [_I, _I, _I, _I]),
    "ruart_gemm_16c_nt_ws": (_I, [_P, _P, _I, _P, _P, _I, _P, _P, _I, _P, _I, _P, _I, _I, _I, _I, _I, _P, _SZ, _I, _P]),
    "ruart_f16c_shifts": (_I, [POINTER(c_int)]),
    "ruart_gemm_16c_set_dual": (_I, [_I]),
    "ruart_bert_set_correction": (_I, [_I, _I, _I, _I, c_ulonglong]),
    "ruart_rows_layernorm_split": (_I, [_P, _I, _P, _P, _F, _P, _P, _P, _I, _I, _I, _P]),
    "ruart_bert_embed_ln_split": (_I, [_P, _P, _P, _P, _P, _P, _P, _F, _P, _P, _P, _I, _I, _I, _P]),
    "ruart_bert_attention_split": (_I, [_P, _I, _P, _P, _I, _I, _I, _I, _P, _P, _P, _P, _P, _P, _P, _P]),
    "ruart_bert_attention_split_set_heads": (_I, [_I]),
    "ruart_gemm_16_nt_splitk": (_I, [_P, _I, _P, _I, _P, _I, _I, _I, _I, _I, _I, _P]),
    "ruart_gemm_16_nt_gelu2": (_I, [_P, _I, _P, _I, _P, _P, _P, _I, _I, _I, _I, _I, _P]),
    "ruart_gemm_16_nt_gelu_bwd_ws_floats": (_SZ, [_I, _I]),
    "ruart_gemm_16_nt_gelu_bwd": (_I, [_P, _I, _P, _I, _P, _I, _P, _P, _I, _P, _I, _I, _I, _P]),
    "ruart_colsum_f32_ws_floats": (_SZ, [_I, _I]),
    "ruart_colsum_f32": (_I, [_P, _I, _I, _I, _P, _I, _P, _P]),
    "ruart_colsum_f32_rows": (_I, [_P, _I, _I, _I, _P, _I, _P]),
    "ruart_gemm_16_tn_splitk": (_I, [_P, _I, _P, _I, _P, _I, _I, _I, _I, _I, _I, _P]),
    "ruart_ln_train_fwd": (_I, [_P, _I, _P, _I, _P, _P, _F, _F, _U, _I, _P, _P, _P, _I, _I, _I, _P]),
    "ruart_ln_train_bwd_ws_floats": (_SZ, [_I]),
    "ruart_ln_train_bwd": (_I, [_P, _I, _P, _P, _P, _I, _P, _P, _F, _U, _I, _P, _I, _P, _I, _P, _P, _P, _I, _P, _I, _I, _P]),
    "ruart_gelu_bwd_rows": (_I, [_P, _P, _I, _P, _P, _I, _I, _P]),
    "ruart_f16_to_bf16": (_I, [_P, _P, _LL, _P]),
    "ruart_weight_prep": (_I, [_P, _I, _F, _P, _I, _P, _I, _I, _I, _P]),
    "ruart_weight_prep_batch": (_I, [POINTER(WPrepItemC), _I, _P]),
    "ruart_colsum_bf16": (_I, [_P, _I, _I, _I, _P, _I, _P, _P]),
    "ruart_transpose16": (_I, [_P, _I, _P, _I, _I, _I, _I, _P]),
    "ruart_splitk_reduce": (_I, [_P, _LL, _I, _P, _LL, _F, _I, _P]),
    "ruart_mix_rows": (_I, [_P, _LL, _I, _I, _P, _P, _I, _I, _I, _P]),
    "ruart_mix_rows_bwd": (_I, [_P, _LL, _I, _I, _P, _I, _P, _P, _I, _I, _P]),
    "ruart_rows_ln_to_16": (_I, [_P, _LL, _I, _P, _LL, _P, _P, _P, _LL, _I, _I, _I, _I, _I, _P]),
    "ruart_attn_train_fwd": (_I, [_P, _I, _P, _I, _I, _I, _I, _P, _P, _P, _F, _U, _P]),
    "ruart_attn_train_bwd": (_I, [_P, _I, _P, _I, _P, _I, _I, _I, _I, _P, _P, _P, _F, _U, _P, _P]),
    "ruart_attn_train_fwd_long": (_I, [_P, _I, _P, _I, _I, _I, _I, _P, _P, _P, _P, _F, _U, _P, _P]),
    "ruart_attn_train_bwd_long": (_I, [_P, _I, _P, _I, _P, _I, _I, _I, _I, _P, _P, _P, _P, _P, _F, _U, _P, _P, _P, _P, _P]),
    "ruart_gemm_f32_nt": (_I, [_P, _I, _P, _I, _P, _P, _I, _P, _I, _I, _I, _I, _I, _P]),
    "ruart_bert_embed_ln": (_I, [_P, _P, _P, _P, _P, _P, _P, _F, _P, _I, _I, _I, _I, _P]),
    "ruart_rows_layernorm": (_I, [_P, _I, _P, _P, _F, _P, _I, _I, _I, _I, _P]),
    "ruart_bert_attention": (_I, [_P, _I, _P, _I, _I, _I, _I, _I, _P, _P, _P, _P, _P, _P, _P, _I, _P, _P, _P, _P, _P]),
    "ruart_bert_pool_set_variant": (_I, [_I]),
    "ruart_bert_pool_mix": (_I, [_P, _LL, _I, _I, _I, _P, _P, _P, _P, _P, _P, _I, _I, _I, _P]),
    "ruart_bert_pool_mix_bwd": (_I, [_P, _LL, _I, _I, _I, _P, _P, _P, _P, _P, _I, _P, _P, _I, _I, _P]),
    "ruart_rows_gather": (_I, [_P, _I, _P, _LL, _P, _LL, _I, _P, _LL, _P, _LL, _I, _P, _LL, _P, _LL, _I, _P]),
    "ruart_cast_f32_to_16": (_I, [_P, _P, _I, _LL, _F, _P]),
    "ruart_bert_workspace_bytes": (_SZ, [POINTER(BertModelC), _I]),
    "ruart_bert_forward": (_I, [POINTER(BertModelC), POINTER(BertBatchC), _P, _P, _SZ, _P]),
    "ruart_bert_workspace_bytes_folded": (_SZ, [POINTER(BertModelC), _I]),
    "ruart_bert_forward_folded": (_I, [POINTER(BertModelC), POINTER(BertBatchC), _P, _P, _P, _SZ, _P]),
    "ruart_gemm_16c_nt_fold": (_I, [_P, _P, _I, _P, _P, _I, _P, _I, _P, _I, _P, _F, _P, _I, _P, _I, _P, _P, _P, _I, _P, _P, _P, _I, _I, _I, _I, _F, _P]),
    "ruart_gemm_16_nt_fold": (_I, [_P, _I, _P, _I, _P, _I, _P, _I, _P, _F, _P, _I, _P, _I, _P, _P, _P, _I, _P, _I, _I, _I, _I, _F, _I, _P]),
    "ruart_rows_stats_finish": (_I, [_P, _I, _I, _F, _F, _P, _P]),
    "ruart_bert_pool_mix_ln": (_I, [_P, _LL, _I, _I, _P, _LL, _P, _P, _P, _P, _P, _P, _P, _P, _I, _I, _I, _P]),
    "ruart_bert_pool_ln_set_variant": (_I, [_I]),
    "ruart_bert_pool_mix_ln_bwd": (_I, [_P, _LL, _I, _I, _P, _LL, _P, _P, _P, _P, _P, _P, _P, _I, _P, _P, _I, _I, _P]),
    "ruart_attn_fwd": (_I, [_P, _P, _P, _P, _P, _I, _I, _P, _P, _I, _I, _I, _I, _I, _P]),
    "ruart_attn_bwd": (_I, [_P, _P, _P, _P, _P, _P, _I, _I, _P, _P, _P, _P, _P, _I, _I, _I, _I, _I, _P]),
    "ruart_attn_set_prefetch": (_I, [_I]),
    "ruart_attn_fwd_pscale": (_I, [_P, _P, _P, _P, _P, _I, _I, _P, _P, _P, _I, _I, _I, _I, _I, _P]),
    "ruart_attn_bwd_pscale": (_I, [_P, _P, _P, _P, _P, _P, _I, _I, _P, _P, _P, _P, _P, _P, _I, _I, _I, _I, _I, _P]),
    "ruart_whole_ln_fwd": (_I, [_P, _P, _P, _P, _LL, _F, _P]),
    "ruart_whole_ln_bwd": (_I, [_P, _P, _P, _P, _P, _LL, _P]),
    "ruart_whole_ln_blocks": (_I, []),
    "ruart_whole_ln_partials": (_I, [_P, _P, _P, _LL, _P]),
    "ruart_whole_ln_var_global": (_I, [_P, _LL, _P, _I, _LL, _P, _P]),
    "ruart_whole_ln_apply_global": (_I, [_P, _P, _LL, _F, _P, _P, _I, _LL, _P, _P]),
    "ruart_whole_ln_bwd_global": (_I, [_P, _P, _P, _P, _LL, _P, _I, _LL, _P]),
    "ruart_scorer_fwd": (_I, [_P, _P, _P, _P, _P, _P, _P, _P, _P, _I, _I, _I, _I, _I, _P]),
    "ruart_scorer_bwd": (_I, [_P, _P, _P, _P, _P, _P, _P, _P, _P, _P, _P, _P, _P, _P, _I, _I, _I, _I, _P]),
    "ruart_scorer_heads_fwd": (_I, [_P, _P, _P, _P, _P, _P, _P, _P, _P, _I, _I, _I, _I, _I, _I, _I, _P]),
    "ruart_scorer_heads_bwd": (_I, [_P, _P, _P, _P, _P, _P, _P, _P, _P, _P, _P, _P, _P, _P, _I, _I, _I, _I, _I, _I, _P]),
    "ruart_lstm_set_variant": (_I, [_I]),
    "ruart_lstm_pack_params": (_I, [_P, _P, _P, _P, _P, _P, _P, _P, _P, _P, _P, _I, _I, _I, _P]),
    "ruart_lstm_ws_bytes": (_I, [_I, _I, POINTER(_SZ)]),
    "ruart_lstm_fwd": (_I, [_P, _P, _P, _P, _P, _P, _I, _I, _I, _I, _P, _SZ, _P]),
    "ruart_lstm_bwd": (_I, [_P, _P, _P, _P, _P, _I, _I, _I, _I, _P, _SZ, _P]),
    "ruart_rows_scale": (_I, [_P, _I, _P, _I, _P, _P, _I, _I, _I, _P]),
    "ruart_lstm_cell_fwd": (_I, [_P, _P, _P, _P, _P, _P, _I, _I, _I, _P]),
    "ruart_lstm_cell_bwd": (_I, [_P, _P, _P, _P, _P, _P, _P, _P, _I, _I, _I, _P]),
    "ruart_set_nan_flag": (_I, [_P]),
    "ruart_grad_norm_clip": (_I, [_P, _P, _P, _P, _I, _F, _P, _P, _P, _P]),
    "ruart_adamax_step": (_I, [_P, _P, _P, _P, _P, _P, _P, _I, _P, _P, _F, _F, _F, _P]),
    "ruart_adam_step": (_I, [_P, _P, _P, _P, _P, _P, _P, _I, _P, _P, _F, _F, _F, _P]),
    "ruart_embedding_bwd_sorted": (_I, [_P, _P, _P, _P, _I, _I, _P, _P]),
    "ruart_embedding_bwd_split": (_I, [_P, _P, _P, _I, _P, _P, _I, _I, _P, _P, _P]),
    "ruart_phoc_table": (_I, [_P, _P, _I, _P, _I, _P, _P]),
    "ruart_edit_distance_pairs": (_I, [_P, _I, _P, _I, _P, _P, _I, _P, _P, _P]),
    "ruart_gemm_bf16_tn": (_I, [_P, _LL, _P, _LL, _P, _I, _I, _I, _I, _P, _SZ, _P]),
    "ruart_gemm_x3_tn_grouped_ws": (_SZ, [POINTER(X3TnProblemC), _I]),
    "ruart_gemm_x3_tn_grouped": (_I, [POINTER(X3TnProblemC), _I, _P, _SZ, _P]),
    "ruart_gemm_x3_plan": (_I, [_I, _I, _I, _I, _I, POINTER(c_int), POINTER(_SZ)]),
    "ruart_gemm_x3": (_I, [_P, _LL, _LL, _P, _LL, _LL, _P, _P, _I, _I, _P, _I, _I,
                           _I, _I, _P, _SZ, _P, _P, _F, _P, _I, _P]),
    "ruart_gemm_x1": (_I, [_P, _LL, _LL, _P, _LL, _LL, _P, _P, _I, _I, _P, _I, _I,
                           _I, _I, _P, _SZ, _P, _P, _F, _P, _I, _P]),
    "ruart_stream_create_cu_masked": (_I, [_I, POINTER(c_void_p)]),
    "ruart_stream_create_priority": (_I, [_I, POINTER(c_void_p)]),
    "ruart_stream_destroy": (_I, [_P]),
    "ruart_gemm_set_tile_order": (_I, [_I]),
    "ruart_gemm_set_variant": (_I, [_I]),
    "ruart_prof_enable": (_I, [_I]),
    "ruart_prof_read": (_I, [POINTER(c_double), POINTER(_LL), POINTER(c_double)]),
    "ruart_prof_mark": (_I, [_I, _P]),
    "ruart_prof_timeline": (_I, [_P, _P, _P, _I, _P]),
}

_UNCHECKED = frozenset({
    "ruart_version", "ruart_gemm_16_tail_ws_bytes", "ruart_gemm_16c_tail_ws_bytes", "ruart_gemm_16_nt_gelu_bwd_ws_floats",
    "ruart_colsum_f32_ws_floats", "ruart_ln_train_bwd_ws_floats", "ruart_bert_workspace_bytes", "ruart_bert_workspace_bytes_folded",
    "ruart_gemm_x3_tn_grouped_ws", "ruart_whole_ln_blocks", "ruart_stream_create_priority", "ruart_gemm_16c_set_dual"})

_lib = _checked = None


class HipError(RuntimeError):
    pass


def _errcheck(rc, fn, args):
    if rc != 0:
        err = HipError("%s failed with hipError_t %d" % (fn.__name__, rc))
        err.code = rc
        raise err
    return rc


def _typed(path, checked):
    lib = ctypes.CDLL(path)
    for name, (res, args) in _SIGNATURES.items():
        fn = getattr(lib, name)
        fn.restype = res
        fn.argtypes = args
        if checked and name not in _UNCHECKED:
            fn.errcheck = _errcheck
    return lib


def load(build_if_missing=True):
    global _lib, _checked
    if _lib is not None:
        return _lib
    if not os.path.exists(LIB_PATH):
        if not build_if_missing:
            raise OSError("libruart_hip.so not built: run `python -m ruart_amd.build`")
        from . import build as _build
        _build.build(verbose=False)
    path = os.environ.get("RUART_HIP_LIB") or LIB_PATH
    lib, checked = _typed(path, False), _typed(path, True)
    if os.environ.get("RUART_GEMM_VARIANT"):
        lib.ruart_gemm_set_variant(int(os.environ["RUART_GEMM_VARIANT"]))
    if os.environ.get("RUART_CORR_DUAL"):
        lib.ruart_gemm_16c_set_dual(int(os.environ["RUART_CORR_DUAL"]))
    _lib, _checked = lib, checked
    return lib


def kernels():
    if _checked is None:
        load()
    return _checked


def exported_symbols():
    return sorted(_SIGNATURES)


def check(rc, what):
    if rc != 0:
        raise HipError("%s failed with hipError_t %d" % (what, rc))


_raw_stream = getattr(torch._C, "_cuda_getCurrentRawStream", None)
_cur_device = getattr(torch._C, "_cuda_getDevice", None)


def stream_handle(device=None):
    if _raw_stream is not None:
        if device is None:
            idx = _cur_device()
        elif isinstance(device, int):
            idx = device
        else:
            idx = device.index if getattr(device, "index", None) is not None else _cur_device()
        return _raw_stream(idx)
    return torch.cuda.current_stream(device).cuda_stream


def stream_ptr(device=None):
    return c_void_p(stream_handle(device))


_DTYPE_CODE = {torch.float32: DT_F32, torch.bfloat16: DT_BF16, torch.float16: DT_F16}


def dtype_code(t):
    return _DTYPE_CODE[t.dtype]


def ptr(t):
    return c_void_p(t.data_ptr()) if t is not None else c_void_p(0)


def f16c_shifts():
    out = (c_int * 4)()
    kernels().ruart_f16c_shifts(out)
    return tuple(int(v) for v in out)


def require_gpu(t, dtype=None):
    if not t.is_cuda:
        raise HipError("ruart_amd kernels need device tensors; got a CPU tensor (there is no CPU fallback)")
    if dtype is not None and t.dtype != dtype:
        raise HipError("expected %s, got %s" % (dtype, t.dtype))
    if not t.is_contiguous():
        raise HipError("tensor must be contiguous")
    return t


def cu_masked_stream(n_cus, device):
    out = c_void_p()
    with torch.cuda.device(device):
        kernels().ruart_stream_create_cu_masked(int(n_cus), ctypes.byref(out))
    st = torch.cuda.ExternalStream(out.value, device=device)
    st._ruart_handle = out.value
    st._ruart_masked = True
    return st


def priority_stream(priority, device):
    out = c_void_p()
    with torch.cuda.device(device):
        rc = load().ruart_stream_create_priority(int(priority), ctypes.byref(out))
    if rc < 0:
        raise HipError("ruart_stream_create_priority failed (%d)" % rc)
    st = torch.cuda.ExternalStream(out.value, device=device)
    st._ruart_handle = out.value
    st._ruart_level = rc
    return st


def destroy_stream(st):
    handle = getattr(st, "_ruart_handle", None)
    if handle is None:
        return
    st.synchronize()
    load().ruart_stream_destroy(handle)
    st._ruart_handle = None
```

Measured before the change: 2882 samples/s.

## Process multiple query/key tiles per block in SDNet attention kernels

Templates the prefetching attention forward, backward-q and backward-kv kernels on a query-tile (QT) or key-tile (KT) count, so one 256-thread block handles up to 4 query or key 16-row tiles. Waves reuse a loaded A or B operand across several MFMAs, and staged K/V panels are amortised over more rows. Mask and probs values are also hoisted into registers. By default the tile count is picked from L1/L2, which means fewer blocks, more LDS per block and more registers, and that may reduce occupancy or parallelism for small batches.

Measured after the change: 2898 samples/s, median of 6. No clear change (+0.6%).

```diff
diff --git a/include/ruart_hip.h b/include/ruart_hip.h
--- a/include/ruart_hip.h
+++ b/include/ruart_hip.h
@@ -195,6 +195,8 @@
                    int diag_len, int relu, float* grad_pa, float* grad_pk, float* grad_v, float* grad_diag_partial,
                    float* ds_ws , int B, int L1, int L2, int h, int D3, void* stream);
 int ruart_attn_set_prefetch(int on);
+int ruart_attn_set_tiles(int query_tiles, int key_tiles);
+int ruart_attn_get_tiles(int* query_tiles, int* key_tiles);
 int ruart_attn_fwd_pscale(const float* pa, const float* pk, const float* v, const unsigned char* mask, const float* diag, int diag_len,
                           int relu, const float* prob_scale, float* out, float* probs, int B, int L1, int L2, int h, int D3,
                           void* stream);
diff --git a/ruart_amd/csrc/sdnet_attention.hip b/ruart_amd/csrc/sdnet_attention.hip
--- a/ruart_amd/csrc/sdnet_attention.hip
+++ b/ruart_amd/csrc/sdnet_attention.hip
@@ -14,6 +14,24 @@
   const int lane = threadIdx.x & 63, r = lane & 15, q = lane >> 4;
   for (int kk = 0; kk < Kc; kk += 4) acc = __builtin_amdgcn_mfma_f32_16x16x4f32(As[r * lda + kk + q], Bs[(kk + q) * sbk + r * sbj], acc, 0, 0, 0);
   return acc;
+}
+template <int N>
+__device__ __forceinline__ void mma16_shared_a(const float* As, int lda, const float* Bs, int tile, int sbk, int sbj, int Kc, f32x4_t* acc) {
+  const int lane = threadIdx.x & 63, r = lane & 15, q = lane >> 4;
+  for (int kk = 0; kk < Kc; kk += 4) {
+    const float av = As[r * lda + kk + q];
+#pragma unroll
+    for (int t = 0; t < N; ++t) acc[t] = __builtin_amdgcn_mfma_f32_16x16x4f32(av, Bs[t * tile + (kk + q) * sbk + r * sbj], acc[t], 0, 0, 0);
+  }
+}
+template <int N>
+__device__ __forceinline__ void mma16_shared_b(const float* As, int tile, int lda, const float* Bs, int sbk, int sbj, int Kc, f32x4_t* acc) {
+  const int lane = threadIdx.x & 63, r = lane & 15, q = lane >> 4;
+  for (int kk = 0; kk < Kc; kk += 4) {
+    const float bv = Bs[(kk + q) * sbk + r * sbj];
+#pragma unroll
+    for (int t = 0; t < N; ++t) acc[t] = __builtin_amdgcn_mfma_f32_16x16x4f32(As[t * tile + r * lda + kk + q], bv, acc[t], 0, 0, 0);
+  }
 }
 
 struct Act {
@@ -347,65 +365,81 @@
   }
 };
 
-template <int UK>
+template <int UK, int QT>
 __global__ __launch_bounds__(256) void attn_fwd_pf_kernel(const float* __restrict__ a, const float* __restrict__ k,
                                                           const float* __restrict__ v, const unsigned char* __restrict__ mask,
                                                           float* __restrict__ out, float* __restrict__ probs, int L1, int L2, int h,
                                                           int D3, int* __restrict__ nan_flag, int relu, const float* __restrict__ diag,
                                                           int diag_len, const float* __restrict__ pscale) {
-  const int b = blockIdx.y, i0 = blockIdx.x * 16;
+  constexpr int QR = 16 * QT;
+  constexpr int WQ = 4 / QT;
+  constexpr int NT = (UK / 4 + WQ - 1) / WQ;
+  const int b = blockIdx.y, i0 = blockIdx.x * QR;
   const int lane = threadIdx.x & 63, wave = threadIdx.x >> 6;
   const int L2p = (L2 + 15) & ~15, ldS = lds_probs_stride(L2p);
   float* a_s = dsm;
-  float* S_s = a_s + 16 * LDA_;
-  float* kv_s = S_s + 16 * ldS;
+  float* S_s = a_s + QR * LDA_;
+  float* kv_s = S_s + QR * ldS;
   const float* ab = a + (size_t)b * L1 * h;
   const float* kb = k + (size_t)b * L2 * h;
   const float* vb = v + (size_t)b * L2 * D3;
   const int ntile = L2p / 16;
-
-  Panel<4, true> pa;
+  const int qt = wave % QT, jw = wave / QT;
+  const int nlive = ntile > jw ? (ntile - jw + WQ - 1) / WQ : 0;
+
+  Panel<4 * QT, true> pa;
   Panel<UK> pk;
-  pa.load(ab, h, 16, i0, L1, 0, h, diag, diag_len);
+  pa.load(ab, h, QR, i0, L1, 0, h, diag, diag_len);
   pk.load(kb, h, L2p, 0, L2, 0, h);
-  f32x4_t acc[NTW];
-#pragma unroll
-  for (int t = 0; t < NTW; ++t) acc[t] = (f32x4_t){0.f, 0.f, 0.f, 0.f};
+  constexpr int NJ = UK / 4;
+  unsigned char mk[NJ];
+#pragma unroll
+  for (int i = 0; i < NJ; ++i) mk[i] = mask[(size_t)b * L2 + min((int)(threadIdx.x & 15) + 16 * i, L2 - 1)];
+  f32x4_t acc[NT];
+#pragma unroll
+  for (int t = 0; t < NT; ++t) acc[t] = (f32x4_t){0.f, 0.f, 0.f, 0.f};
   for (int c0 = 0; c0 < h; c0 += CH) {
     __syncthreads();
-    pa.store(a_s, LDA_, 16, relu);
+    pa.store(a_s, LDA_, QR, relu);
     pk.store(kv_s, LDA_, L2p, relu);
     {
       const bool more = c0 + CH < h;
-      pa.load(ab, h, 16, i0, L1, more ? c0 + CH : 0, h, diag, diag_len);
+      pa.load(ab, h, QR, i0, L1, more ? c0 + CH : 0, h, diag, diag_len);
       pk.load(more ? kb : vb, more ? h : D3, L2p, 0, L2, more ? c0 + CH : 0, more ? h : D3);
     }
     __syncthreads();
     const int kc = min(CH, (h - c0 + 3) & ~3);
-#pragma unroll
-    for (int t = 0; t < NTW; ++t) {
-      const int jt = wave + 4 * t;
-      if (jt < ntile) acc[t] = mma16(a_s, LDA_, kv_s + jt * 16 * LDA_, 1, LDA_, kc, acc[t]);
-    }
-  }
-#pragma unroll
-  for (int t = 0; t < NTW; ++t) {
-    const int jt = wave + 4 * t;
+    if (nlive == NT) {
+      mma16_shared_a<NT>(a_s + qt * 16 * LDA_, LDA_, kv_s + jw * 16 * LDA_, WQ * 16 * LDA_, 1, LDA_, kc, acc);
+    } else {
+#pragma unroll
+      for (int t = 0; t < NT; ++t)
+        if (t < nlive) acc[t] = mma16(a_s + qt * 16 * LDA_, LDA_, kv_s + (jw + WQ * t) * 16 * LDA_, 1, LDA_, kc, acc[t]);
+    }
+  }
+#pragma unroll
+  for (int t = 0; t < NT; ++t) {
+    const int jt = jw + WQ * t;
     if (jt < ntile) {
 #pragma unroll
-      for (int r = 0; r < 4; ++r) S_s[((lane >> 4) * 4 + r) * ldS + jt * 16 + (lane & 15)] = acc[t][r];
+      for (int r = 0; r < 4; ++r) S_s[(qt * 16 + (lane >> 4) * 4 + r) * ldS + jt * 16 + (lane & 15)] = acc[t][r];
     }
   }
   __syncthreads();
-  {
-    const int row = threadIdx.x >> 4, c = threadIdx.x & 15;
-    const unsigned char* mb = mask + (size_t)b * L2;
+  bool bad = false;
+  for (int g = 0; g < QT; ++g) {
+    if (i0 + g * 16 >= L1) break;
+    const int row = g * 16 + (threadIdx.x >> 4), c = threadIdx.x & 15;
     float* Sr = S_s + row * ldS;
     float mx = -INFINITY;
-    for (int j = c; j < L2; j += 16) {
-      const float s = mb[j] ? Sr[j] : -INFINITY;
-      Sr[j] = s;
-      mx = fmaxf(mx, s);
+#pragma unroll
+    for (int i = 0; i < NJ; ++i) {
+      const int j = c + 16 * i;
+      if (j < L2) {
+        const float s = mk[i] ? Sr[j] : -INFINITY;
+        Sr[j] = s;
+        mx = fmaxf(mx, s);
+      }
     }
 #pragma unroll
     for (int o = 8; o > 0; o >>= 1) mx = fmaxf(mx, __shfl_xor(mx, o, 64));
@@ -419,7 +453,6 @@
     for (int o = 8; o > 0; o >>= 1) sum += __shfl_xor(sum, o, 64);
     const float inv = 1.0f / sum;
     const bool live = (i0 + row) < L1;
-    bool bad = false;
     for (int j = c; j < L2p; j += 16) {
       const float p = (j < L2) ? Sr[j] * inv : 0.f;
       const float ps = (pscale && live && j < L2) ? pscale[((size_t)b * L1 + i0 + row) * L2 + j] : 1.f;
@@ -427,96 +460,123 @@
       bad |= live && !(p == p);
       if (probs && live && j < L2) probs[((size_t)b * L1 + i0 + row) * L2 + j] = p;
     }
-    if (bad && nan_flag) atomicOr(nan_flag, 1);
-  }
+  }
+  if (bad && nan_flag) atomicOr(nan_flag, 1);
   for (int d0 = 0; d0 < D3; d0 += CH) {
     __syncthreads();
     pk.store(kv_s, LDB_, L2p, 0);
     pk.load(vb, D3, L2p, 0, L2, d0 + CH < D3 ? d0 + CH : 0, D3);
     __syncthreads();
-    f32x4_t o = {0.f, 0.f, 0.f, 0.f};
-    o = mma16(S_s, ldS, kv_s + wave * 16, LDB_, 1, L2p, o);
     const int d = d0 + wave * 16 + (lane & 15);
-#pragma unroll
-    for (int r = 0; r < 4; ++r) {
-      const int i = i0 + (lane >> 4) * 4 + r;
-      if (i < L1 && d < D3) out[((size_t)b * L1 + i) * D3 + d] = o[r];
-    }
-  }
-}
-
-template <int UK>
+    f32x4_t o[QT];
+#pragma unroll
+    for (int q = 0; q < QT; ++q) o[q] = (f32x4_t){0.f, 0.f, 0.f, 0.f};
+    mma16_shared_b<QT>(S_s, 16 * ldS, ldS, kv_s + wave * 16, LDB_, 1, L2p, o);
+#pragma unroll
+    for (int q = 0; q < QT; ++q) {
+#pragma unroll
+      for (int r = 0; r < 4; ++r) {
+        const int i = i0 + q * 16 + (lane >> 4) * 4 + r;
+        if (i < L1 && d < D3) out[((size_t)b * L1 + i) * D3 + d] = o[q][r];
+      }
+    }
+  }
+}
+
+template <int UK, int QT>
 __global__ __launch_bounds__(256) void attn_bwd_q_pf_kernel(const float* __restrict__ k, const float* __restrict__ v,
                                                             const float* __restrict__ probs, const float* __restrict__ gout,
                                                             float* __restrict__ grad_a, float* __restrict__ dS, int L1, int L2, int h,
                                                             int D3, const float* __restrict__ pa_, int relu,
                                                             const float* __restrict__ diag, int diag_len,
                                                             float* __restrict__ grad_diag, const float* __restrict__ pscale) {
-  const int b = blockIdx.y, i0 = blockIdx.x * 16;
+  constexpr int QR = 16 * QT, WQ = 4 / QT, NT = (UK / 4 + WQ - 1) / WQ;
+  const int b = blockIdx.y, i0 = blockIdx.x * QR;
   const int lane = threadIdx.x & 63, wave = threadIdx.x >> 6;
   const int L2p = (L2 + 15) & ~15, ldS = lds_probs_stride(L2p);
   float* g_s = dsm;
-  float* S_s = g_s + 16 * LDA_;
-  float* kv_s = S_s + 16 * ldS;
+  float* S_s = g_s + QR * LDA_;
+  float* kv_s = S_s + QR * ldS;
   const float* kb = k + (size_t)b * L2 * h;
   const float* vb = v + (size_t)b * L2 * D3;
   const float* gb = gout + (size_t)b * L1 * D3;
-  const int ntile = L2p / 16;
-
-  Panel<4> pg;
+  const int ntile = L2p / 16, nqt = (L1 + 15) / 16;
+  const int qt = wave % QT, jw = wave / QT;
+  const int nlive = ntile > jw ? (ntile - jw + WQ - 1) / WQ : 0;
+
+  Panel<4 * QT> pg;
   Panel<UK> pk;
-  pg.load(gb, D3, 16, i0, L1, 0, D3);
+  pg.load(gb, D3, QR, i0, L1, 0, D3);
   pk.load(vb, D3, L2p, 0, L2, 0, D3);
-  f32x4_t acc[NTW];
-#pragma unroll
-  for (int t = 0; t < NTW; ++t) acc[t] = (f32x4_t){0.f, 0.f, 0.f, 0.f};
+  f32x4_t acc[NT];
+#pragma unroll
+  for (int t = 0; t < NT; ++t) acc[t] = (f32x4_t){0.f, 0.f, 0.f, 0.f};
   for (int c0 = 0; c0 < D3; c0 += CH) {
     __syncthreads();
-    pg.store(g_s, LDA_, 16, 0);
+    pg.store(g_s, LDA_, QR, 0);
     pk.store(kv_s, LDA_, L2p, 0);
     {
       const bool more = c0 + CH < D3;
-      pg.load(gb, D3, 16, i0, L1, more ? c0 + CH : 0, D3);
+      pg.load(gb, D3, QR, i0, L1, more ? c0 + CH : 0, D3);
       pk.load(more ? vb : kb, more ? D3 : h, L2p, 0, L2, more ? c0 + CH : 0, more ? D3 : h);
     }
     __syncthreads();
     const int kc = min(CH, (D3 - c0 + 3) & ~3);
-#pragma unroll
-    for (int t = 0; t < NTW; ++t) {
-      const int jt = wave + 4 * t;
-      if (jt < ntile) acc[t] = mma16(g_s, LDA_, kv_s + jt * 16 * LDA_, 1, LDA_, kc, acc[t]);
-    }
-  }
-#pragma unroll
-  for (int t = 0; t < NTW; ++t) {
-    const int jt = wave + 4 * t;
+    if (nlive == NT) {
+      mma16_shared_a<NT>(g_s + qt * 16 * LDA_, LDA_, kv_s + jw * 16 * LDA_, WQ * 16 * LDA_, 1, LDA_, kc, acc);
+    } else {
+#pragma unroll
+      for (int t = 0; t < NT; ++t)
+        if (t < nlive) acc[t] = mma16(g_s + qt * 16 * LDA_, LDA_, kv_s + (jw + WQ * t) * 16 * LDA_, 1, LDA_, kc, acc[t]);
+    }
+  }
+  constexpr int NJ = UK / 4;
+  float pr[QT][NJ];
+#pragma unroll
+  for (int g = 0; g < QT; ++g) {
+    const int i = i0 + g * 16 + (int)(threadIdx.x >> 4);
+    const float* Pr = probs + ((size_t)b * L1 + (i < L1 ? i : 0)) * L2;
+#pragma unroll
+    for (int u = 0; u < NJ; ++u) pr[g][u] = Pr[min((int)(threadIdx.x & 15) + 16 * u, L2 - 1)];
+  }
+#pragma unroll
+  for (int t = 0; t < NT; ++t) {
+    const int jt = jw + WQ * t;
     if (jt < ntile) {
 #pragma unroll
-      for (int r = 0; r < 4; ++r) S_s[((lane >> 4) * 4 + r) * ldS + jt * 16 + (lane & 15)] = acc[t][r];
+      for (int r = 0; r < 4; ++r) S_s[(qt * 16 + (lane >> 4) * 4 + r) * ldS + jt * 16 + (lane & 15)] = acc[t][r];
     }
   }
   __syncthreads();
-  {
-    const int row = threadIdx.x >> 4, c = threadIdx.x & 15;
+#pragma unroll
+  for (int g = 0; g < QT; ++g) {
+    if (i0 + g * 16 >= L1) break;
+    const int row = g * 16 + (threadIdx.x >> 4), c = threadIdx.x & 15;
     const bool live = (i0 + row) < L1;
-    const float* Pr = probs + ((size_t)b * L1 + (live ? i0 + row : 0)) * L2;
     float* Sr = S_s + row * ldS;
     float dot = 0.f;
     if (pscale && live) {
       const float* Mr = pscale + ((size_t)b * L1 + i0 + row) * L2;
       for (int j = c; j < L2; j += 16) Sr[j] *= Mr[j];
     }
-    for (int j = c; j < L2; j += 16) dot += Sr[j] * Pr[j];
+#pragma unroll
+    for (int i = 0; i < NJ; ++i) {
+      const int j = c + 16 * i;
+      if (j < L2) dot += Sr[j] * pr[g][i];
+    }
 #pragma unroll
     for (int o = 8; o > 0; o >>= 1) dot += __shfl_xor(dot, o, 64);
-    for (int j = c; j < L2p; j += 16) {
-      float d = 0.f;
-      if (live && j < L2) {
-        const float p = Pr[j];
-        d = p * (Sr[j] - dot);
-        dS[((size_t)b * L1 + i0 + row) * L2 + j] = d;
+#pragma unroll
+    for (int i = 0; i < NJ; ++i) {
+      const int j = c + 16 * i;
+      if (j < L2p) {
+        float d = 0.f;
+        if (live && j < L2) {
+          d = pr[g][i] * (Sr[j] - dot);
+          dS[((size_t)b * L1 + i0 + row) * L2 + j] = d;
+        }
+        Sr[j] = d;
       }
-      Sr[j] = d;
     }
   }
   for (int d0 = 0; d0 < h; d0 += CH) {
@@ -524,42 +584,49 @@
     pk.store(kv_s, LDB_, L2p, relu);
     pk.load(kb, h, L2p, 0, L2, d0 + CH < h ? d0 + CH : 0, h);
     __syncthreads();
-    f32x4_t o = {0.f, 0.f, 0.f, 0.f};
-    o = mma16(S_s, ldS, kv_s + wave * 16, LDB_, 1, L2p, o);
     const int d = d0 + wave * 16 + (lane & 15);
-    float gd = 0.f;
     const float dsc = (d < h) ? (diag_len == 1 ? diag[0] : (diag_len > 1 ? diag[d] : 1.f)) : 0.f;
-#pragma unroll
-    for (int r = 0; r < 4; ++r) {
-      const int i = i0 + (lane >> 4) * 4 + r;
-      if (i < L1 && d < h) {
-        const size_t at = ((size_t)b * L1 + i) * h + d;
-        float g = o[r];
-        if (pa_) {
-          const float pv = pa_[at];
-          gd += g * (relu ? fmaxf(pv, 0.f) : pv);
-          g = (relu && pv <= 0.f) ? 0.f : g * dsc;
+    f32x4_t o[QT];
+#pragma unroll
+    for (int q = 0; q < QT; ++q) o[q] = (f32x4_t){0.f, 0.f, 0.f, 0.f};
+    mma16_shared_b<QT>(S_s, 16 * ldS, ldS, kv_s + wave * 16, LDB_, 1, L2p, o);
+#pragma unroll
+    for (int q = 0; q < QT; ++q) {
+      if (i0 + q * 16 >= L1) break;
+      float gd = 0.f;
+#pragma unroll
+      for (int r = 0; r < 4; ++r) {
+        const int i = i0 + q * 16 + (lane >> 4) * 4 + r;
+        if (i < L1 && d < h) {
+          const size_t at = ((size_t)b * L1 + i) * h + d;
+          float g = o[q][r];
+          if (pa_) {
+            const float pv = pa_[at];
+            gd += g * (relu ? fmaxf(pv, 0.f) : pv);
+            g = (relu && pv <= 0.f) ? 0.f : g * dsc;
+          }
+          grad_a[at] = g;
         }
-        grad_a[at] = g;
       }
-    }
-    if (grad_diag) {
-      gd += __shfl_xor(gd, 16, 64);
-      gd += __shfl_xor(gd, 32, 64);
-      if ((lane >> 4) == 0 && d < h) grad_diag[((size_t)b * gridDim.x + blockIdx.x) * h + d] = gd;
-    }
-  }
-}
-
+      if (grad_diag) {
+        gd += __shfl_xor(gd, 16, 64);
+        gd += __shfl_xor(gd, 32, 64);
+        if ((lane >> 4) == 0 && d < h) grad_diag[((size_t)b * nqt + blockIdx.x * QT + q) * h + d] = gd;
+      }
+    }
+  }
+}
+
+template <int KT>
 struct PanelT16 {
-  float v[4], m[4];
+  float v[4 * KT], m[4 * KT];
   unsigned ok;
   __device__ __forceinline__ void load(const float* __restrict__ src, int ld, int r0, int rows, int c0, int cols, const float* __restrict__ mul) {
     ok = 0;
 #pragma unroll
-    for (int u = 0; u < 4; ++u) {
+    for (int u = 0; u < 4 * KT; ++u) {
       const int e = (int)threadIdx.x + u * 256;
-      const int c = e & 15, r = e >> 4;
+      const int c = e % (16 * KT), r = e / (16 * KT);
       const int gr = r0 + r, gc = c0 + c;
       if (gr < rows && gc < cols) ok |= 1u << u;
       const size_t at = (size_t)min(gr, rows - 1) * ld + min(gc, cols - 1);
@@ -569,22 +636,25 @@
   }
   __device__ __forceinline__ void store(float* dst, int ldd) const {
 #pragma unroll
-    for (int u = 0; u < 4; ++u) {
+    for (int u = 0; u < 4 * KT; ++u) {
       const int e = (int)threadIdx.x + u * 256;
-      dst[(e & 15) * ldd + (e >> 4)] = ((ok >> u) & 1u) ? v[u] * m[u] : 0.f;
+      dst[(e % (16 * KT)) * ldd + e / (16 * KT)] = ((ok >> u) & 1u) ? v[u] * m[u] : 0.f;
     }
   }
 };
 
+template <int KT>
 __device__ __forceinline__ void tn_product_pf(const float* X, int L1, int L2, int j0, const float* Y, int N, float* C, float* xt_s,
                                               float* y_s, Act yact, const float* out_gate, const float* xmul) {
   const int lane = threadIdx.x & 63, wave = threadIdx.x >> 6;
   const int nr = (L1 + CH - 1) / CH, nn = (N + CH - 1) / CH, steps = nr * nn;
-  PanelT16 px;
+  PanelT16<KT> px;
   Panel<16, true> py;
   px.load(X, L2, 0, L1, j0, L2, xmul);
   py.load(Y, N, CH, 0, L1, 0, N, yact.diag, yact.diag_len);
-  f32x4_t o = {0.f, 0.f, 0.f, 0.f};
+  f32x4_t o[KT];
+#pragma unroll
+  for (int t = 0; t < KT; ++t) o[t] = (f32x4_t){0.f, 0.f, 0.f, 0.f};
   int ri = 0, ni = 0;
   for (int s = 0; s < steps; ++s) {
     const int r0 = ri * CH, n0 = ni * CH;
@@ -598,38 +668,42 @@
     py.load(Y, N, CH, rn * CH, L1, nx * CH, N, yact.diag, yact.diag_len);
     __syncthreads();
     const int kc = min(CH, (L1 - r0 + 3) & ~3);
-    o = mma16(xt_s, LDA_, y_s + wave * 16, LDB_, 1, kc, o);
+    mma16_shared_b<KT>(xt_s, 16 * LDA_, LDA_, y_s + wave * 16, LDB_, 1, kc, o);
     if (ri == nr - 1) {
       const int n = n0 + wave * 16 + (lane & 15);
 #pragma unroll
-      for (int r = 0; r < 4; ++r) {
-        const int j = j0 + (lane >> 4) * 4 + r;
-        if (j < L2 && n < N) {
-          const size_t at = (size_t)j * N + n;
-          C[at] = (out_gate && out_gate[at] <= 0.f) ? 0.f : o[r];
+      for (int t = 0; t < KT; ++t) {
+#pragma unroll
+        for (int r = 0; r < 4; ++r) {
+          const int j = j0 + t * 16 + (lane >> 4) * 4 + r;
+          if (j < L2 && n < N) {
+            const size_t at = (size_t)j * N + n;
+            C[at] = (out_gate && out_gate[at] <= 0.f) ? 0.f : o[t][r];
+          }
         }
+        o[t] = (f32x4_t){0.f, 0.f, 0.f, 0.f};
       }
-      o = (f32x4_t){0.f, 0.f, 0.f, 0.f};
     }
     ri = rn;
     ni = nx;
   }
 }
 
+template <int KT>
 __global__ __launch_bounds__(256) void attn_bwd_kv_pf_kernel(const float* __restrict__ a, const float* __restrict__ probs,
                                                              const float* __restrict__ dS, const float* __restrict__ gout,
                                                              float* __restrict__ grad_k, float* __restrict__ grad_v, int L1, int L2, int h,
                                                              int D3, const float* __restrict__ pk, int relu,
                                                              const float* __restrict__ diag, int diag_len,
                                                              const float* __restrict__ pscale) {
-  const int b = blockIdx.y, j0 = blockIdx.x * 16;
+  const int b = blockIdx.y, j0 = blockIdx.x * 16 * KT;
   float* xt_s = dsm;
-  float* y_s = xt_s + 16 * LDA_;
+  float* y_s = xt_s + 16 * KT * LDA_;
   const size_t pb = (size_t)b * L1 * L2;
-  tn_product_pf(dS + pb, L1, L2, j0, a + (size_t)b * L1 * h, h, grad_k + (size_t)b * L2 * h, xt_s, y_s, Act{relu, diag, diag_len},
-                (relu && pk) ? pk + (size_t)b * L2 * h : nullptr, nullptr);
-  tn_product_pf(probs + pb, L1, L2, j0, gout + (size_t)b * L1 * D3, D3, grad_v + (size_t)b * L2 * D3, xt_s, y_s, no_act(), nullptr,
-                pscale ? pscale + pb : nullptr);
+  tn_product_pf<KT>(dS + pb, L1, L2, j0, a + (size_t)b * L1 * h, h, grad_k + (size_t)b * L2 * h, xt_s, y_s, Act{relu, diag, diag_len},
+                    (relu && pk) ? pk + (size_t)b * L2 * h : nullptr, nullptr);
+  tn_product_pf<KT>(probs + pb, L1, L2, j0, gout + (size_t)b * L1 * D3, D3, grad_v + (size_t)b * L2 * D3, xt_s, y_s, no_act(), nullptr,
+                    pscale ? pscale + pb : nullptr);
 }
 
 #define WLN_BLOCKS 256
@@ -845,18 +919,32 @@
 
 static bool g_attn_prefetch = !(getenv("RUART_ATTN_PREFETCH") && atoi(getenv("RUART_ATTN_PREFETCH")) == 0);
 template <typename K> static void attn_big_lds(K kern) { hipFuncSetAttribute((const void*)kern, hipFuncAttributeMaxDynamicSharedMemorySize, 160 * 1024); }
+template <int U> static void attn_big_lds_pf() {
+  attn_big_lds(attn_fwd_pf_kernel<U, 1>), attn_big_lds(attn_fwd_pf_kernel<U, 2>), attn_big_lds(attn_fwd_pf_kernel<U, 4>);
+  attn_big_lds(attn_bwd_q_pf_kernel<U, 1>), attn_big_lds(attn_bwd_q_pf_kernel<U, 2>), attn_big_lds(attn_bwd_q_pf_kernel<U, 4>);
+}
 static void attn_allow_big_lds() {
-  static bool done = (attn_big_lds(attn_fwd_kernel), attn_big_lds(attn_bwd_q_kernel), attn_big_lds(attn_fwd_pf_kernel<12>),
-                      attn_big_lds(attn_fwd_pf_kernel<16>), attn_big_lds(attn_fwd_pf_kernel<28>), attn_big_lds(attn_fwd_pf_kernel<32>),
-                      attn_big_lds(attn_bwd_q_pf_kernel<12>), attn_big_lds(attn_bwd_q_pf_kernel<16>), attn_big_lds(attn_bwd_q_pf_kernel<28>),
-                      attn_big_lds(attn_bwd_q_pf_kernel<32>), true);
+  static bool done = (attn_big_lds(attn_fwd_kernel), attn_big_lds(attn_bwd_q_kernel), attn_big_lds_pf<12>(), attn_big_lds_pf<16>(),
+                      attn_big_lds_pf<28>(), attn_big_lds_pf<32>(), true);
   (void)done;
 }
 
-static size_t attn_lds_bytes(int L2) {
+static size_t attn_lds_bytes(int L2, int qt = 1) {
   const int L2p = (L2 + 15) & ~15;
   const int ldS = ((L2p + 31) / 32) * 32 + 2;
-  return sizeof(float) * (size_t)(16 * LDA_ + 16 * ldS + L2p * LDB_);
+  return sizeof(float) * (size_t)(16 * qt * LDA_ + 16 * qt * ldS + L2p * LDB_);
+}
+
+static int g_attn_qt = 0, g_attn_kt = 0;
+static int attn_query_tiles(int L1) {
+  int q = g_attn_qt ? g_attn_qt : 4;
+  while (q > 1 && 16 * (q / 2) >= L1) q /= 2;
+  return q;
+}
+static int attn_key_tiles(int L2p) {
+  const int nt = L2p / 16;
+  if (g_attn_kt) return g_attn_kt < nt ? g_attn_kt : nt;
+  return ceil_div(nt, ceil_div(nt, 4));
 }
 
 __global__ __launch_bounds__(256) void attn1_fwd_kernel(const float* __restrict__ a, const float* __restrict__ k,
@@ -991,8 +1079,11 @@
   const dim3 grid(ceil_div(L1, 16), B), block(256);
   attn_allow_big_lds();
   const int L2p = (L2 + 15) & ~15;
-#define RUART_AF(U) hipLaunchKernelGGL(attn_fwd_pf_kernel<U>, grid, block, attn_lds_bytes(L2), (hipStream_t)stream, a, k, v, mask, out, probs, \
-                                       L1, L2, h, D3, ruart_nan_flag_ptr, relu, diag_len ? diag : nullptr, diag_len, prob_scale)
+  const int qt = attn_query_tiles(L1);
+#define RUART_AF_Q(U, Q) hipLaunchKernelGGL((attn_fwd_pf_kernel<U, Q>), dim3(ceil_div(L1, 16 * Q), B), block, attn_lds_bytes(L2, Q),              \
+                                            (hipStream_t)stream, a, k, v, mask, out, probs, L1, L2, h, D3, ruart_nan_flag_ptr, relu,            \
+                                            diag_len ? diag : nullptr, diag_len, prob_scale)
+#define RUART_AF(U) do { if (qt == 4) RUART_AF_Q(U, 4); else if (qt == 2) RUART_AF_Q(U, 2); else RUART_AF_Q(U, 1); } while (0)
   if (!g_attn_prefetch || L2p > 128)
     hipLaunchKernelGGL(attn_fwd_kernel, grid, block, attn_lds_bytes(L2), (hipStream_t)stream, a, k, v, mask, out, probs, L1, L2, h, D3,
                        ruart_nan_flag_ptr, relu, diag_len ? diag : nullptr, diag_len, prob_scale);
@@ -1001,6 +1092,7 @@
   else if (L2p <= 112) RUART_AF(28);
   else RUART_AF(32);
 #undef RUART_AF
+#undef RUART_AF_Q
   RUART_CHECK_LAUNCH();
   return 0;
 }
@@ -1008,6 +1100,23 @@
 extern "C" int ruart_attn_set_prefetch(int on) {
   RUART_ENTRY();
   g_attn_prefetch = on != 0;
+  return 0;
+}
+
+extern "C" int ruart_attn_set_tiles(int query_tiles, int key_tiles) {
+  RUART_ENTRY();
+  if ((query_tiles != 0 && query_tiles != 1 && query_tiles != 2 && query_tiles != 4) || key_tiles < 0 || key_tiles > 4)
+    return (int)hipErrorInvalidValue;
+  g_attn_qt = query_tiles;
+  g_attn_kt = key_tiles;
+  return 0;
+}
+
+extern "C" int ruart_attn_get_tiles(int* query_tiles, int* key_tiles) {
+  RUART_ENTRY();
+  if (!query_tiles || !key_tiles) return (int)hipErrorInvalidValue;
+  *query_tiles = g_attn_qt;
+  *key_tiles = g_attn_kt;
   return 0;
 }
 
@@ -1036,9 +1145,11 @@
   const float* dg = diag_len ? diag : nullptr;
   attn_allow_big_lds();
   const int L2p = (L2 + 15) & ~15;
-#define RUART_AQ(U) hipLaunchKernelGGL(attn_bwd_q_pf_kernel<U>, dim3(ceil_div(L1, 16), B), dim3(256), attn_lds_bytes(L2), (hipStream_t)stream, \
-                                       k, v, probs, grad_out, grad_a, ds_ws, L1, L2, h, D3, act ? a : nullptr, relu, dg, diag_len,           \
-                                       (diag_len > 1) ? grad_diag : nullptr, prob_scale)
+  const int qt = attn_query_tiles(L1);
+#define RUART_AQ_Q(U, Q) hipLaunchKernelGGL((attn_bwd_q_pf_kernel<U, Q>), dim3(ceil_div(L1, 16 * Q), B), dim3(256), attn_lds_bytes(L2, Q),        \
+                                            (hipStream_t)stream, k, v, probs, grad_out, grad_a, ds_ws, L1, L2, h, D3, act ? a : nullptr, relu,  \
+                                            dg, diag_len, (diag_len > 1) ? grad_diag : nullptr, prob_scale)
+#define RUART_AQ(U) do { if (qt == 4) RUART_AQ_Q(U, 4); else if (qt == 2) RUART_AQ_Q(U, 2); else RUART_AQ_Q(U, 1); } while (0)
   if (!g_attn_prefetch || L2p > 128)
     hipLaunchKernelGGL(attn_bwd_q_kernel, dim3(ceil_div(L1, 16), B), dim3(256), attn_lds_bytes(L2), (hipStream_t)stream, k, v, probs,
                        grad_out, grad_a, ds_ws, L1, L2, h, D3, act ? a : nullptr, relu, dg, diag_len,
@@ -1048,14 +1159,23 @@
   else if (L2p <= 112) RUART_AQ(28);
   else RUART_AQ(32);
 #undef RUART_AQ
+#undef RUART_AQ_Q
   RUART_CHECK_LAUNCH();
   const size_t lds = sizeof(float) * (16 * LDA_ + CH * LDB_);
-  if (g_attn_prefetch)
-    hipLaunchKernelGGL(attn_bwd_kv_pf_kernel, dim3(ceil_div(L2, 16), B), dim3(256), lds, (hipStream_t)stream, a, probs, ds_ws, grad_out,
-                       grad_k, grad_v, L1, L2, h, D3, k, relu, dg, diag_len, prob_scale);
-  else
+#define RUART_AKV(T) hipLaunchKernelGGL(attn_bwd_kv_pf_kernel<T>, dim3(ceil_div(L2p, 16 * T), B), dim3(256),                              \
+                                        sizeof(float) * (16 * T * LDA_ + CH * LDB_), (hipStream_t)stream, a, probs, ds_ws, grad_out,     \
+                                        grad_k, grad_v, L1, L2, h, D3, k, relu, dg, diag_len, prob_scale)
+  if (g_attn_prefetch) {
+    const int kt = attn_key_tiles(L2p);
+    if (kt == 4) RUART_AKV(4);
+    else if (kt == 3) RUART_AKV(3);
+    else if (kt == 2) RUART_AKV(2);
+    else RUART_AKV(1);
+  } else {
     hipLaunchKernelGGL(attn_bwd_kv_kernel, dim3(ceil_div(L2, 16), B), dim3(256), lds, (hipStream_t)stream, a, probs, ds_ws, grad_out,
                        grad_k, grad_v, L1, L2, h, D3, k, relu, dg, diag_len, prob_scale);
+  }
+#undef RUART_AKV
   RUART_CHECK_LAUNCH();
   return 0;
 }
diff --git a/ruart_amd/hip.py b/ruart_amd/hip.py
--- a/ruart_amd/hip.py
+++ b/ruart_amd/hip.py
@@ -125,6 +125,8 @@
     "ruart_attn_fwd": (_I, [_P, _P, _P, _P, _P, _I, _I, _P, _P, _I, _I, _I, _I, _I, _P]),
     "ruart_attn_bwd": (_I, [_P, _P, _P, _P, _P, _P, _I, _I, _P, _P, _P, _P, _P, _I, _I, _I, _I, _I, _P]),
     "ruart_attn_set_prefetch": (_I, [_I]),
+    "ruart_attn_set_tiles": (_I, [_I, _I]),
+    "ruart_attn_get_tiles": (_I, [POINTER(c_int), POINTER(c_int)]),
     "ruart_attn_fwd_pscale": (_I, [_P, _P, _P, _P, _P, _I, _I, _P, _P, _P, _I, _I, _I, _I, _I, _P]),
     "ruart_attn_bwd_pscale": (_I, [_P, _P, _P, _P, _P, _P, _I, _I, _P, _P, _P, _P, _P, _P, _I, _I, _I, _I, _I, _P]),
     "ruart_whole_ln_fwd": (_I, [_P, _P, _P, _P, _LL, _F, _P]),
@@ -219,6 +221,8 @@
         lib.ruart_gemm_set_variant(int(os.environ["RUART_GEMM_VARIANT"]))
     if os.environ.get("RUART_CORR_DUAL"):
         lib.ruart_gemm_16c_set_dual(int(os.environ["RUART_CORR_DUAL"]))
+    if os.environ.get("RUART_ATTN_TILES"):
+        check(lib.ruart_attn_set_tiles(*(int(x) for x in os.environ["RUART_ATTN_TILES"].split(","))), "ruart_attn_set_tiles")
     _lib, _checked = lib, checked
     return lib
 
```
